# YangGuang001/siddhi

Hardware: AMD Instinct MI355X
Metric: input events/sec (node) for partitioned pattern query; achieved HBM GB/s % (higher is better)
Workload: dtype f32+i64

## Files before the change

### siddhi_amd/abi.py

```python
import ctypes as C

SH_DESC_VERSION = 5
SH_MAX_ORDER = 4
SH_MAX_GROUP = 4

SH_OK = 0
SH_E_INVALID_ARG = -1
SH_E_OOM = -2
SH_E_HIP = -3
SH_E_UNSUPPORTED = -4
SH_E_STATE_OVERFLOW = -5
SH_E_MORE = -6
SH_E_NO_DEVICE = -7

STATUS_NAMES = {0: "OK", -1: "INVALID_ARG", -2: "OOM", -3: "HIP", -4: "UNSUPPORTED",
                -5: "STATE_OVERFLOW", -6: "MORE", -7: "NO_DEVICE"}


class sh_expr(C.Structure):
    _fields_ = [("op", C.c_int32), ("type", C.c_int32), ("lhs", C.c_int32), ("rhs", C.c_int32),
                ("third", C.c_int32), ("ltype", C.c_int32), ("rtype", C.c_int32),
                ("slot", C.c_int32), ("chain", C.c_int32), ("attr", C.c_int32),
                ("is_null", C.c_int32), ("pad", C.c_int32), ("cval", C.c_int64)]

# ... 59 lines not shown


class sh_due_cand(C.Structure):
    _fields_ = [("t", C.c_int64), ("order", C.c_uint64), ("key", C.c_int32), ("pad", C.c_int32)]


HISTORY_FN = C.CFUNCTYPE(C.c_int, C.c_void_p, C.POINTER(C.c_uint64), C.c_int64,
                         C.POINTER(C.POINTER(C.c_uint64)), C.POINTER(C.c_int64))
SELECT_FN = C.CFUNCTYPE(C.c_int, C.c_void_p, C.c_int32, C.POINTER(sh_due_cand), C.c_int64,
                        C.POINTER(C.c_int64), C.POINTER(C.c_int64))
MIN_TIME_FN = C.CFUNCTYPE(C.c_int, C.c_void_p, C.c_int64, C.POINTER(C.c_int64))


class sh_coordinator(C.Structure):
    _fields_ = [("user", C.c_void_p), ("history", HISTORY_FN), ("select", SELECT_FN), ("min_time", MIN_TIME_FN)]


class sh_kernel_times(C.Structure):
    _fields_ = [("segment_ms", C.c_float), ("advance_ms", C.c_float), ("emit_ms", C.c_float),
                ("total_ms", C.c_float), ("advance_launches", C.c_int64)]


EXPORTED = ["sh_start", "sh_compile", "sh_push_batch", "sh_advance_time", "sh_drain", "sh_pending",
            "sh_destroy", "sh_last_error", "sh_run_device", "sh_run_device_v2", "sh_last_kernel_times",
            "sh_version", "sh_device_count", "sh_set_partition_keys", "sh_snapshot", "sh_restore",
            "sh_set_coordinator", "sh_push_batch_part", "sh_drain_ordered", "sh_list_get",
            "sh_packed_row_layout"]


def bind_product(lib):
    lib.sh_compile.argtypes = [C.POINTER(sh_app_desc), C.POINTER(C.c_void_p)]
    lib.sh_compile.restype = C.c_int
    lib.sh_start.argtypes = [C.c_void_p]
    lib.sh_start.restype = C.c_int
    lib.sh_push_batch.argtypes = [C.c_void_p, C.POINTER(sh_batch)]
    lib.sh_push_batch.restype = C.c_int
    lib.sh_advance_time.argtypes = [C.c_void_p, C.c_int64]
    lib.sh_advance_time.restype = C.c_int
    lib.sh_drain.argtypes = [C.c_void_p, C.POINTER(sh_match_buf)]
    lib.sh_drain.restype = C.c_int
    lib.sh_pending.argtypes = [C.c_void_p]
    lib.sh_pending.restype = C.c_int64
    lib.sh_destroy.argtypes = [C.c_void_p]
    lib.sh_destroy.restype = None
    lib.sh_last_error.argtypes = [C.c_void_p]
    lib.sh_last_error.restype = C.c_char_p
    lib.sh_set_partition_keys.argtypes = [C.c_void_p, C.c_int32, C.c_int32, C.c_void_p, C.c_void_p]
    lib.sh_set_partition_keys.restype = C.c_int
    lib.sh_run_device.argtypes = [C.c_void_p, C.POINTER(sh_device_run)]
    lib.sh_run_device.restype = C.c_int
    lib.sh_run_device_v2.argtypes = [C.c_void_p, C.POINTER(sh_device_run)]
    lib.sh_run_device_v2.restype = C.c_int
    lib.sh_last_kernel_times.argtypes = [C.c_void_p, C.POINTER(sh_kernel_times)]
    lib.sh_last_kernel_times.restype = C.c_int
    lib.sh_packed_row_layout.argtypes = [C.c_void_p, C.POINTER(C.c_int32), C.c_int32, C.POINTER(C.c_int32),
                                         C.POINTER(C.c_int32)]
    lib.sh_packed_row_layout.restype = C.c_int
    lib.sh_snapshot.argtypes = [C.c_void_p, C.c_void_p, C.c_int64, C.POINTER(C.c_int64)]
    lib.sh_snapshot.restype = C.c_int
    lib.sh_restore.argtypes = [C.c_void_p, C.c_void_p, C.c_int64]
    lib.sh_restore.restype = C.c_int
    lib.sh_set_coordinator.argtypes = [C.c_void_p, C.POINTER(sh_coordinator)]
    lib.sh_set_coordinator.restype = C.c_int
    lib.sh_push_batch_part.argtypes = [C.c_void_p, C.POINTER(sh_batch), C.c_void_p, C.c_int64, C.c_int64]
    lib.sh_push_batch_part.restype = C.c_int
    lib.sh_drain_ordered.argtypes = [C.c_void_p, C.POINTER(sh_match_buf), C.c_void_p]
    lib.sh_drain_ordered.restype = C.c_int
    lib.sh_list_get.argtypes = [C.c_void_p, C.c_int64, C.c_int64, C.c_void_p, C.c_void_p]
    lib.sh_list_get.restype = C.c_int64
    lib.sh_version.argtypes = []
    lib.sh_version.restype = C.c_char_p
    lib.sh_device_count.argtypes = []
    lib.sh_device_count.restype = C.c_int
    lib.shx_jit_status.argtypes = [C.c_void_p]
    lib.shx_jit_status.restype = C.c_int
    lib.shx_jit_compile.argtypes = [C.c_void_p]
    lib.shx_jit_compile.restype = C.c_int
    lib.shx_jit_source.argtypes = [C.c_void_p, C.c_char_p, C.c_int64]
    lib.shx_jit_source.restype = C.c_int64
    lib.shx_bucket_compile.argtypes = [C.c_void_p, C.c_char_p, C.c_int64]
    lib.shx_bucket_compile.restype = C.c_int
    lib.shx_bucket_status.argtypes = [C.c_void_p]
    lib.shx_bucket_status.restype = C.c_int
    lib.shx_bucket_emit_status.argtypes = [C.c_void_p]
    lib.shx_bucket_emit_status.restype = C.c_int
    lib.shx_emit_compile.argtypes = [C.c_void_p, C.c_int, C.c_char_p, C.c_int64]
    lib.shx_emit_compile.restype = C.c_int
    lib.shx_emit_compile_key.argtypes = [C.POINTER(C.c_int32), C.c_char_p, C.c_int64, C.c_char_p, C.c_int64]
    lib.shx_emit_compile_key.restype = C.c_int
    lib.shx_seq3_status.argtypes = [C.c_void_p]
    lib.shx_seq3_status.restype = C.c_int
    lib.shx_agg_status.argtypes = [C.c_void_p]
    lib.shx_agg_status.restype = C.c_int
    lib.shx_having_status.argtypes = [C.c_void_p]
    lib.shx_having_status.restype = C.c_int
    lib.shx_having_rows.argtypes = [C.c_void_p, C.POINTER(C.c_int64), C.POINTER(C.c_int64)]
    lib.shx_having_rows.restype = C.c_int
    lib.shx_having_ms.argtypes = [C.c_void_p]
    lib.shx_having_ms.restype = C.c_double
    lib.shx_rate_status.argtypes = [C.c_void_p]
    lib.shx_rate_status.restype = C.c_int
    lib.shx_rate_rows.argtypes = [C.c_void_p, C.POINTER(C.c_int64), C.POINTER(C.c_int64)]
    lib.shx_rate_rows.restype = C.c_int
    lib.shx_rate_ms.argtypes = [C.c_void_p]
    lib.shx_rate_ms.restype = C.c_double
    lib.shx_fingerprint.argtypes = [C.c_void_p]
    lib.shx_fingerprint.restype = C.c_uint64
    lib.shx_rules_status.argtypes = [C.c_void_p]
    lib.shx_rules_status.restype = C.c_int
    lib.shx_rules_carry.argtypes = [C.c_void_p, C.POINTER(C.c_int64), C.POINTER(C.c_int64)]
    lib.shx_rules_carry.restype = C.c_int
    lib.shx_rules_agg_carry.argtypes = [C.c_void_p, C.POINTER(C.c_int64)]
    lib.shx_rules_agg_carry.restype = C.c_int
    lib.shx_rules_agg_capacity.argtypes = [C.c_void_p]
    lib.shx_rules_agg_capacity.restype = C.c_int64
    lib.shx_host_profile.argtypes = [C.c_void_p, C.c_void_p, C.c_void_p, C.c_int]
    lib.shx_host_profile.restype = C.c_int
    lib.shx_seq3_shape.argtypes = [C.c_void_p]
    lib.shx_seq3_shape.restype = C.c_int
    return lib


def bind_oracle(lib):
    lib.ref_create.argtypes = [C.POINTER(sh_app_desc), C.c_char_p, C.c_int]
    lib.ref_create.restype = C.c_void_p
    lib.ref_start.argtypes = [C.c_void_p]
    lib.ref_start.restype = None
    lib.ref_send.argtypes = [C.c_void_p, C.POINTER(sh_batch), C.c_uint64]
    lib.ref_send.restype = C.c_int
    lib.ref_set_partition_keys.argtypes = [C.c_void_p, C.c_int32, C.c_int32, C.c_void_p, C.c_void_p]
    lib.ref_set_partition_keys.restype = C.c_int
    lib.ref_advance_time.argtypes = [C.c_void_p, C.c_int64]
    lib.ref_advance_time.restype = C.c_int
    lib.ref_out_count.argtypes = [C.c_void_p]
    lib.ref_out_count.restype = C.c_int64
    lib.ref_out_read.argtypes = [C.c_void_p, C.c_int64, C.c_int64, C.c_void_p, C.c_void_p,
                                 C.c_void_p, C.c_void_p, C.c_void_p, C.c_int32, C.c_void_p]
    lib.ref_out_read.restype = C.c_int
    lib.ref_out_clear.argtypes = [C.c_void_p]
    lib.ref_out_clear.restype = None
    lib.ref_list_get.argtypes = [C.c_void_p, C.c_int64, C.c_int64, C.c_void_p, C.c_void_p]
    lib.ref_list_get.restype = C.c_int64
    lib.ref_destroy.argtypes = [C.c_void_p]
    lib.ref_destroy.restype = None
    return lib


def object_columns(compiled):
    return [[k for k, t in enumerate(q.out_types) if t == 6] for q in compiled.queries]


def resolve_lists(out, obj_cols, get):
    import numpy as np
    lists = {}
    if any(obj_cols):
        q = out["query"]
        for r in range(len(q)):
            cols = obj_cols[int(q[r])] if 0 <= int(q[r]) < len(obj_cols) else []
            for c in cols:
                if not out["nulls"][r, c]:
                    v, nl = get(int(out["values"][r, c]))
                    lists[(r, c)] = (np.asarray(v, np.int64), np.asarray(nl, np.uint8))
    out["lists"] = lists
    return out


# ... 26 lines not shown
```

### siddhi_amd/build.py

```python
import os
import subprocess
import sys

HERE = os.path.dirname(os.path.abspath(__file__))
CSRC = os.path.join(HERE, "csrc")
OUT = os.path.join(HERE, "libsiddhi_hip.so")
SOURCES = ["sh_host.cpp", "sh_host_nfa.cpp", "sh_host_fast.cpp", "sh_host_snap.cpp", "sh_jit.cpp", "sh_nfa_lower.cpp", "sh_kernels.hip", "sh_window.hip", "sh_nfa.hip", "sh_rules.hip", "sh_bucket.hip", "sh_shard.hip", "sh_agg.hip", "sh_having.hip", "sh_rate.hip"]
JIT_HEADERS = [os.path.join(HERE, "..", "include", "sh_query.h"), os.path.join(CSRC, "sh_program.h"),
               os.path.join(CSRC, "sh_device.h"), os.path.join(CSRC, "sh_vm.h"),
               os.path.join(CSRC, "sh_wave.h")]
JIT_EMIT_HEADERS = [os.path.join(CSRC, "sh_rows.h"), os.path.join(CSRC, "sh_bk_emit.h")]
JIT_INC = os.path.join(CSRC, "sh_jit_src.inc")
JIT_PRELUDE = """typedef __hip_internal::int8_t int8_t;
typedef __hip_internal::uint8_t uint8_t;
typedef __hip_internal::int16_t int16_t;
typedef __hip_internal::uint16_t uint16_t;
typedef __hip_internal::int32_t int32_t;
typedef __hip_internal::uint32_t uint32_t;
typedef __hip_internal::int64_t int64_t;
typedef __hip_internal::uint64_t uint64_t;
typedef decltype(sizeof(0)) size_t;
#define INT32_MIN (-2147483647 - 1)
#define INT64_MIN (-9223372036854775807LL - 1)
"""
FLAGS = ["-O3", "-std=c++17", "-fPIC", "-shared", "--offload-arch=gfx950", "-ffp-contract=off",
         "-fno-gpu-flush-denormals-to-zero", "-fhip-fp32-correctly-rounded-divide-sqrt",
         "-Wall", "-Wno-unused-function", "-Wno-unused-result", "-Wno-unused-value", "-L/opt/rocm/lib", "-lhiprtc", "-Wl,-rpath,/opt/rocm/lib"]


def _jit_text(headers, prelude=""):
    parts = [prelude]
    for h in headers:
        with open(h) as f:
            for line in f:
                t = line.strip()
                if t.startswith("#include") or t == "#pragma once":
                    continue
                parts.append(line)
    text = "".join(parts)
    assert ')SHJ"' not in text
    return text


def write_jit_inc():
    inc = "// generated by siddhi_amd/build.py from the device headers -- do not edit\n" \
          "static const char SHJ_HEADERS[] = R\"SHJ(" + _jit_text(JIT_HEADERS, JIT_PRELUDE) + ")SHJ\";\n" \
          "static const char SHJ_EMIT_SRC[] = R\"SHJ(" + _jit_text(JIT_EMIT_HEADERS) + ")SHJ\";\n"
    if os.path.exists(JIT_INC) and open(JIT_INC).read() == inc:
        return
    with open(JIT_INC, "w") as f:
        f.write(inc)


def needs_build():
    if not os.path.exists(OUT):
        return True
    t = os.path.getmtime(OUT)
    deps = [os.path.join(CSRC, f) for f in os.listdir(CSRC)] + \
        [os.path.join(HERE, "..", "include", f) for f in os.listdir(os.path.join(HERE, "..", "include"))]
    return any(os.path.getmtime(d) > t for d in deps)


OBJ_DIR = os.path.join(HERE, "build")
COMPILE_FLAGS = [f for f in FLAGS if f not in ("-shared",) and not f.startswith(("-L", "-l", "-Wl"))]
LINK_FLAGS = ["-shared", "-fPIC", "--offload-arch=gfx950", "-L/opt/rocm/lib", "-lhiprtc", "-Wl,-rpath,/opt/rocm/lib"]


def _headers_mtime():
    hs = [os.path.join(CSRC, f) for f in os.listdir(CSRC) if f.endswith((".h", ".inc"))] + \
        [os.path.join(HERE, "..", "include", f) for f in os.listdir(os.path.join(HERE, "..", "include"))]
    return max(os.path.getmtime(h) for h in hs)


def build(force=False, verbose=False):
    write_jit_inc()
    if not force and not needs_build():
        return OUT
    from concurrent.futures import ThreadPoolExecutor
    hipcc = os.environ.get("HIPCC", "/opt/rocm/bin/hipcc")
    os.makedirs(OBJ_DIR, exist_ok=True)
    hmt = _headers_mtime()
    objs, jobs = [], []
    for src in SOURCES:
        sp = os.path.join(CSRC, src)
        op = os.path.join(OBJ_DIR, src + ".o")
        objs.append(op)
        if force or not os.path.exists(op) or os.path.getmtime(op) < max(os.path.getmtime(sp), hmt):
            jobs.append([hipcc] + COMPILE_FLAGS + ["-c", sp, "-o", op])

    def run(cmd):
        if verbose:
            print(" ".join(cmd), file=sys.stderr)
# ... 14 lines not shown
```

### siddhi_amd/csrc/sh_bk_emit.h

```cpp
#pragma once
#include <hip/hip_runtime.h>
#include <stdint.h>

#include "../../include/sh_query.h"
#include "sh_device.h"
#include "sh_rows.h"
#include "sh_wave.h"

#define BK_TPB 512
#define BK_ITEMS (SHB_TILE / BK_TPB)

static_assert(BK_ITEMS == 16, "tile / threads");


__device__ __forceinline__ int bk_tile(int nt) {
    const int per = (nt + 7) >> 3;
    const int t = (int)(blockIdx.x & 7u) * per + (int)(blockIdx.x >> 3);
    return t < nt ? t : -1;
}
__device__ __forceinline__ int bk_tile(int t0, int t1) {
    const int t = bk_tile(t1 - t0);
    return t < 0 ? -1 : t0 + t;
}

// ... 23 lines not shown
        bk_vals<NO>(O, i, mp, row, v);
        bk_store<MODE, NO>(OC, row, v, seq, out_seq, out_vals);
        return;
    }
#ifndef BKS_NO
    const int no = O.n_out;
    if (MODE == SHB_OUT_PACKED) {
        uint32_t* r = (uint32_t*)OC.rows + row * OC.rw;
        r[0] = (uint32_t)seq;
        r[1] = (uint32_t)(seq >> 32);
        for (int k = 2; k < OC.rw; k++) r[k] = 0u;
    } else if (out_seq) {
        out_seq[row] = seq;
    }
    for (int o = 0; o < no; o++) {
        const int64_t v = bk_raw(o_src[o], o_kind[o] == 1 ? i : mp, o_type[o]);
        if (MODE == SHB_OUT_PACKED) {
            uint32_t* r = (uint32_t*)OC.rows + row * OC.rw + OC.woff[o];
            r[0] = OC.colw[o] == 1 ? (uint32_t)(uint8_t)v : (uint32_t)v;
            if (OC.colw[o] == 8) r[1] = (uint32_t)((uint64_t)v >> 32);
        } else if (MODE == SHB_OUT_COLS) {
            bk_put(OC.cols[o], OC.colw[o], row, v);
        } else if (out_vals) {
            out_vals[row * no + o] = v;
        }
    }
#endif
}

#ifdef BKS_NO
extern "C" __global__ void __launch_bounds__(BK_TPB, BKS_OCC) BKS_NAME(shb_plan P, bks_ptrs Q, uint64_t seq_base,
                                                               uint64_t* __restrict__ out_seq,
                                                               int64_t* __restrict__ out_vals, int64_t out_cap) {
    constexpr int MODE = BKS_MODE, NO = BKS_NO, BK_RU = BKS_RU, BK_OCC = BKS_OCC;
    const bks_ptrs &O = Q, &OC = Q;
#else
template <int MODE, int NO, int BK_RU, int BK_OCC = 4>
__global__ void __launch_bounds__(BK_TPB, BK_OCC) k_bk_emit(shb_plan P, shb_out O, shb_cols OC, uint64_t seq_base,
                                                    uint64_t* __restrict__ out_seq, int64_t* __restrict__ out_vals,
                                                    int64_t out_cap) {
#endif
    constexpr bool LM = BK_OCC >= 6;
    constexpr int EROWS = LM ? 512 : BK_EROWS;
    constexpr int EMPW = LM ? 2 * BK_EHALF : BK_EHALF;
    constexpr int BK_MAPW = (BK_TPB / 64) * (EROWS / 2 + EMPW + BK_EHALF / 2);
    __shared__ uint32_t pool[(SHB_TILE + 1) > BK_MAPW ? (SHB_TILE + 1) : BK_MAPW];
    uint32_t* const pfx = pool;
    uint16_t(*const rmap)[EROWS] = (uint16_t(*)[EROWS])pool;
    uint32_t(*const emp)[EMPW] = (uint32_t(*)[EMPW])(pool + (BK_TPB / 64) * (EROWS / 2));
    uint16_t(*const ero)[BK_EHALF] =
        (uint16_t(*)[BK_EHALF])(pool + (BK_TPB / 64) * (EROWS / 2 + EMPW));
    __shared__ uint32_t ms0[SHB_NB];
    __shared__ uint16_t to[SHB_NB + 1];
    __shared__ uint32_t wtot[BK_TPB / 64], ws[BK_TPB / 64];
    __shared__ int32_t o_kind[SHB_MAX_OUT], o_type[SHB_MAX_OUT];
    __shared__ const void* o_src[SHB_MAX_OUT];
    __shared__ uint32_t s_tb;
    constexpr int NV = NO > 0 ? NO : 1;
    const int T = bk_tile(P.et0, P.et1);
    if (T < 0) return;
    const int64_t b0 = (int64_t)T << SHB_TILE_SHIFT;
    const int tile_n = (int)((P.n - b0) < SHB_TILE ? (P.n - b0) : SHB_TILE);
    const int lane = threadIdx.x & 63, w = threadIdx.x >> 6;
    if (threadIdx.x <= SHB_NB) to[threadIdx.x] = P.toff[(int64_t)T * SHB_TOFF + threadIdx.x];
    if (threadIdx.x < SHB_NB) ms0[threadIdx.x] = P.mstart[(int64_t)T * SHB_NB + threadIdx.x];
    if (threadIdx.x == 0) s_tb = P.ttot[T];
#ifndef BKS_NO
    if (NO == 0 && threadIdx.x < SHB_MAX_OUT) {
#pragma unroll
        for (int o = 0; o < SHB_MAX_OUT; o++)
            if (o == (int)threadIdx.x) {
                o_kind[o] = O.kind[o];
                o_type[o] = O.type[o];
                o_src[o] = O.src[o];
            }
    }
#endif
    uint32_t sl[BK_ITEMS];
    {
        const int l0 = w * (64 * BK_ITEMS) + lane;
#pragma unroll
        for (int j = 0; j < BK_ITEMS; j++) {
            const int l = l0 + j * 64;
            sl[j] = l < tile_n ? (uint32_t)P.sp[b0 + l] : BK_NOSLOT;
        }
    }
    {
        const int s0 = threadIdx.x * 16;
        const uint4 q = *(const uint4*)(P.cnt + b0 + s0);
        __syncthreads();
        const int nv = to[SHB_NB];
        uint32_t c[16];
        const uint32_t wd[4] = {q.x, q.y, q.z, q.w};
        uint32_t sum = 0;
#pragma unroll
        for (int k = 0; k < 16; k++) {
            c[k] = (s0 + k < nv) ? (wd[k >> 2] >> (8 * (k & 3))) & 0xFFu : 0u;
            sum += c[k];
        }
        uint32_t tot;
        uint32_t off = shw_block_excl<BK_TPB>(sum, ws, &tot);
        int d = 0;
        {
            int lo = 0, hi = SHB_NB - 1;
            while (lo < hi) {
                const int mid = (lo + hi + 1) >> 1;
                if ((int)to[mid] <= s0) lo = mid;
                else hi = mid - 1;
            }
            d = lo;
        }
#pragma unroll
        for (int k = 0; k < 16; k++) {
            while (d < SHB_NB - 1 && (int)to[d + 1] <= s0 + k) d++;
            pfx[s0 + k] = off | ((uint32_t)d << BK_PFX_BITS);
            off += c[k];
        }
        if (threadIdx.x == 0) pfx[SHB_TILE] = tot;
        __syncthreads();
    }
    uint32_t cp[BK_ITEMS / 4];
    uint32_t mp[BK_ITEMS];
    uint32_t mine = 0;
#pragma unroll
    for (int j = 0; j < BK_ITEMS; j++) {
        uint32_t c = 0;
        mp[j] = 0u;
        if (sl[j] != BK_NOSLOT) {
            const uint32_t s = sl[j];
            const uint32_t pw = pfx[s];
            const uint32_t d = pw >> BK_PFX_BITS;
            const uint32_t ps = pw & BK_PFX_MASK;
            c = (pfx[s + 1] & BK_PFX_MASK) - ps;
            mp[j] = ms0[d] + ps - (pfx[to[d]] & BK_PFX_MASK);
        }
        if ((j & 3) == 0) cp[j >> 2] = 0u;
        cp[j >> 2] |= c << (8 * (j & 3));
        mine += c;
    }
    {
        const uint32_t wsum = shw_last(shw_incl_scan(mine));
        if (lane == 0) wtot[w] = wsum;
    }
    __syncthreads();
    if (LM) {
#pragma unroll
        for (int j = 0; j < BK_ITEMS; j++) emp[w][j * 64 + lane] = mp[j];
    }
    uint64_t rb = s_tb;
    for (int q = 0; q < w; q++) rb += wtot[q];
#pragma unroll
    for (int hf = 0; hf < BK_ITEMS / 8; hf++) {
        uint32_t carry = 0;
        uint32_t ro8[8];
#pragma unroll
        for (int jj = 0; jj < 8; jj++) {
            const int j = hf * 8 + jj;
            const uint32_t c = (cp[j >> 2] >> (8 * (j & 3))) & 0xFFu;
            const uint32_t incl = shw_incl_scan(c);
            const uint32_t ro = carry + incl - c;
            if (!LM) ro8[jj] = ro;
            const int e = jj * 64 + lane;
            if (!LM) emp[w][e] = mp[j];
            ero[w][e] = (uint16_t)ro;
            for (uint32_t k = 0; k < c; k++)
                if (ro + k < EROWS) rmap[w][ro + k] = (uint16_t)e;
            carry += shw_last(incl);
// ... 74 lines not shown
```

### siddhi_amd/csrc/sh_bucket.hip

```cpp
#include <hip/hip_runtime.h>
#include <stdlib.h>
#include <string.h>

#include "../../include/sh_query.h"
#include "sh_device.h"
#include "sh_nfa.h"
#include "sh_bk_emit.h"
#include "sh_rows.h"
#include "sh_wave.h"

static inline unsigned bk_grid(int nt) { return 8u * (unsigned)((nt + 7) >> 3); }


template <int MINW, int TPB>
__global__ void __launch_bounds__(TPB, MINW) k_bk_scatter(const int32_t* __restrict__ keys,
                                                          const int64_t* __restrict__ ts, int32_t nkeys, shb_plan P) {
    constexpr int SC_ITEMS = SHB_TILE / TPB;
    __shared__ uint32_t wcnt[TPB / 64][256];
    __shared__ uint32_t tstart[256];
    __shared__ uint32_t ws[TPB / 64];
    __shared__ uint32_t stage[SHB_TILE];
    __shared__ int64_t s_tmx[TPB / 64];
    const int T = bk_tile(P.nt);
    if (T < 0) return;
    const int64_t b0 = (int64_t)T << SHB_TILE_SHIFT;
    const int lane = threadIdx.x & 63, w = threadIdx.x >> 6;
    for (int c = threadIdx.x; c < (TPB / 64) * 256; c += TPB) (&wcnt[0][0])[c] = 0u;
    __syncthreads();
    int32_t key[SC_ITEMS];
    uint32_t rw[SC_ITEMS], wp[SC_ITEMS];
    const uint64_t lt = lane ? (~0ull >> (64 - lane)) : 0ull;
    {
        int64_t tv[SC_ITEMS];
        const int64_t e0 = b0 + (int64_t)w * (64 * SC_ITEMS) + lane;
        if (b0 + SHB_TILE <= P.n) {
            const int32_t* __restrict__ pk = keys + e0;
            const int64_t* __restrict__ pt = ts + e0;
#pragma unroll
            for (int j = 0; j < SC_ITEMS; j++) {
                key[j] = pk[j * 64];
                tv[j] = pt[j * 64];
            }
        } else {
#pragma unroll
            for (int j = 0; j < SC_ITEMS; j++) {
                const int64_t i = e0 + j * 64;
                const bool in = i < P.n;
                key[j] = in ? keys[i] : -1;
                tv[j] = in ? ts[i] : P.tbase;
            }
        }
        const int64_t lim = (int64_t)1 << (32 - P.kb);
        bool bad = false, badk = false;
        int64_t tmx = INT64_MIN;
#pragma unroll
        for (int j = 0; j < SC_ITEMS; j++) {
            const int64_t dt = tv[j] - P.tbase;
            if (key[j] >= nkeys) badk = true;
            if (key[j] >= 0 && !P.no_ts && (dt < 0 || dt >= lim)) bad = true;
            if (key[j] >= 0 && tv[j] > tmx) tmx = tv[j];
            wp[j] = P.no_ts ? ((uint32_t)key[j] >> 8) : (((uint32_t)dt << P.kb) | ((uint32_t)key[j] >> 8));
            rw[j] = key[j] >= 0 ? ((uint32_t)key[j] & (SHB_NB - 1)) << 16 : ~0u;
        }
        if (bad) atomicOr(P.flag, SHB_F_TS);
        if (badk) atomicOr(P.flag, SHB_F_KEY);
#pragma unroll
        for (int o = 32; o >= 1; o >>= 1) {
            const int64_t y = __shfl_xor(tmx, o);
            tmx = y > tmx ? y : tmx;
        }
        if (lane == 0) s_tmx[w] = tmx;
        if (threadIdx.x == 0) P.tfirst[T] = tv[0];
    }
    {
        uint32_t old[SC_ITEMS];
#pragma unroll
        for (int j = 0; j < SC_ITEMS; j++) {
            const bool valid = rw[j] != ~0u;
            const uint32_t d = (rw[j] >> 16) & (SHB_NB - 1);
            uint64_t peers = __ballot(valid);
#pragma unroll
            for (int bb = 0; bb < 8; bb++) {
                const bool bit = (d >> bb) & 1u;
                const uint64_t m = __ballot(valid && bit);
                peers &= bit ? m : ~m;
            }
            const uint32_t r = (uint32_t)__popcll(peers & lt);
            old[j] = 0u;
            if (valid && r == 0) old[j] = atomicAdd(&wcnt[w][d], (uint32_t)__popcll(peers));
            rw[j] = valid ? (r | ((uint32_t)(__ffsll((unsigned long long)peers) - 1) << 8) | (d << 16)) : ~0u;
        }
#pragma unroll
        for (int j = 0; j < SC_ITEMS; j++) {
            const uint32_t ld = rw[j] == ~0u ? (uint32_t)lane : (rw[j] >> 8) & 63u;
            const uint32_t base = (uint32_t)__shfl((int)old[j], (int)ld);
            if (rw[j] != ~0u) rw[j] = ((base + (rw[j] & 0xFFu)) & 0xFFFFu) | (rw[j] & 0xFF0000u);
        }
    }
    __syncthreads();
    uint32_t nvalid;
    {
        uint32_t tot = 0;
        if (threadIdx.x < 256) {
#pragma unroll
            for (int q = 0; q < TPB / 64; q++) {
                const uint32_t c = wcnt[q][threadIdx.x];
                wcnt[q][threadIdx.x] = tot;
                tot += c;
            }
        }
        const uint32_t ex = shw_block_excl<TPB>(threadIdx.x < 256 ? tot : 0u, ws, &nvalid);
        if (threadIdx.x < 256) {
            tstart[threadIdx.x] = ex;
            P.toff[(int64_t)T * SHB_TOFF + threadIdx.x] = (uint16_t)ex;
        }
        if (threadIdx.x == 256) P.toff[(int64_t)T * SHB_TOFF + 256] = (uint16_t)nvalid;
        if (threadIdx.x == 0) {
            int64_t m = s_tmx[0];
#pragma unroll
            for (int q = 1; q < TPB / 64; q++) m = s_tmx[q] > m ? s_tmx[q] : m;
            P.tpre[T] = m;
        }
    }
    __syncthreads();
#pragma unroll
    for (int j = 0; j < SC_ITEMS; j++) {
        const bool valid = rw[j] != ~0u;
        const uint32_t d = (rw[j] >> 16) & (SHB_NB - 1);
        rw[j] = valid ? tstart[d] + wcnt[w][d] + (rw[j] & 0xFFFFu) : ~0u;
        const int64_t i = b0 + (int64_t)w * (64 * SC_ITEMS) + j * 64 + lane;
        if (i < P.n) P.sp[i] = (uint16_t)rw[j];
        if (valid) stage[rw[j]] = wp[j];
    }
    __syncthreads();
    const int64_t ob = (int64_t)T << SHB_TILE_SHIFT;
#define BK_WRITE_OUT(TY, DST, EXPR)                                                  \
    {                                                                                \
        _Pragma("unroll 4") for (int m = 0; m < SC_ITEMS; m++) {                     \
            const uint32_t l = (uint32_t)(m * TPB + threadIdx.x);                 \
            if (l < nvalid) ((TY*)(DST))[EXPR(ob + l)] = (TY)stage[l];               \
        }                                                                            \
        __syncthreads();                                                             \
    }
#define BK_ID(x) (x)
#define BK_LO(x) (2 * (x))
#define BK_HI(x) (2 * (x) + 1)
    BK_WRITE_OUT(uint32_t, P.w0, BK_ID);
    for (int c = 0; c < P.n_staged; c++) {
        const int wd = P.st_width[c];
        const int halves = wd == 8 ? 2 : 1;
        for (int hh = 0; hh < halves; hh++) {
#pragma unroll
            for (int j = 0; j < SC_ITEMS; j++) {
                if (rw[j] == ~0u) continue;
                const int64_t i = b0 + (int64_t)w * (64 * SC_ITEMS) + j * 64 + lane;
                uint32_t v;
                if (wd == 8) v = ((const uint32_t*)P.st_src[c])[2 * i + hh];
                else if (wd == 4) v = ((const uint32_t*)P.st_src[c])[i];
                else v = ((const uint8_t*)P.st_src[c])[i];
                stage[rw[j]] = v;
            }
            __syncthreads();
            if (wd == 8) {
                if (hh == 0) BK_WRITE_OUT(uint32_t, P.st_dst[c], BK_LO)
                else BK_WRITE_OUT(uint32_t, P.st_dst[c], BK_HI)
            } else if (wd == 4) {
                BK_WRITE_OUT(uint32_t, P.st_dst[c], BK_ID)
            } else {
                BK_WRITE_OUT(uint8_t, P.st_dst[c], BK_ID)
            }
        }
    }
#undef BK_WRITE_OUT
#undef BK_ID
#undef BK_LO
#undef BK_HI
}


__device__ __forceinline__ void bk_halo(const int64_t* __restrict__ tfirst, int32_t* __restrict__ hstart, int32_t nt,
                                        int64_t within, int t) {
    if (t >= nt) return;
    const int64_t ta = tfirst[t];
    const int64_t tlim = ta < INT64_MIN + within ? INT64_MIN : ta - within;
    int h = t > 0 ? 1 : 0;
    while (h < t && h < SHB_HMAX && tfirst[t - h] >= tlim) h++;
    hstart[t] = t - h;
}

__device__ __forceinline__ void bk_tpre(int64_t* __restrict__ tpre, int32_t nt, int64_t* s) {
    const int per = (nt + 1023) / 1024;
    const int t0 = threadIdx.x * per;
    int64_t m = INT64_MIN;
    for (int t = t0; t < t0 + per && t < nt; t++) m = tpre[t] > m ? tpre[t] : m;
    s[threadIdx.x] = m;
    __syncthreads();
    for (int o = 1; o < 1024; o <<= 1) {
        const int64_t y = threadIdx.x >= (unsigned)o ? s[threadIdx.x - o] : INT64_MIN;
        __syncthreads();
        if (y > s[threadIdx.x]) s[threadIdx.x] = y;
        __syncthreads();
    }
    int64_t run = threadIdx.x ? s[threadIdx.x - 1] : INT64_MIN;
    for (int t = t0; t < t0 + per && t < nt; t++) {
        const int64_t v = tpre[t];
        tpre[t] = run;
        run = v > run ? v : run;
    }
}

#define S3B_TPB 1024
#define S3B_CH 4096
#define S3B_NR (S3B_CH / S3B_TPB)
#define S3B_NK 4096
#define S3B_W (S3B_TPB / 64)

__device__ __forceinline__ NfVal s3b_val(uint32_t b, int t) {
    NfVal v;
    v.t = (uint8_t)t;
    v.null = 0;
    v.b = t == SH_T_INT ? (int64_t)(int32_t)b : (int64_t)b;
    return v;
}

__device__ __forceinline__ void s3b_sort_pass(const uint32_t* __restrict__ c_key, const uint16_t* in,
                                              uint16_t* out, int L, int sh, uint32_t (*wc)[64], uint32_t* ws) {
    const int lane = threadIdx.x & 63, w = threadIdx.x >> 6;
    const uint64_t lt = lane ? (~0ull >> (64 - lane)) : 0ull;
    for (int c = threadIdx.x; c < S3B_W * 64; c += S3B_TPB) (&wc[0][0])[c] = 0u;
    __syncthreads();
    uint32_t rk[S3B_NR], dg[S3B_NR], ix[S3B_NR];
#pragma unroll
    for (int r = 0; r < S3B_NR; r++) {
        const int pos = (w * S3B_NR + r) * 64 + lane;
        const bool valid = pos < L;
        ix[r] = valid ? (in ? (uint32_t)in[pos] : (uint32_t)pos) : 0u;
        const uint32_t d = valid ? (c_key[ix[r]] >> sh) & 63u : 0u;
        uint64_t peers = __ballot(valid);
#pragma unroll
        for (int bb = 0; bb < 6; bb++) {
            const bool bit = (d >> bb) & 1u;
            const uint64_t m = __ballot(valid && bit);
            peers &= bit ? m : ~m;
        }
        const uint32_t r_ = (uint32_t)__popcll(peers & lt);
        const uint32_t base = valid ? wc[w][d] : 0u;
        if (valid && r_ == 0) wc[w][d] = base + (uint32_t)__popcll(peers);
        rk[r] = valid ? base + r_ : ~0u;
        dg[r] = d;
    }
    __syncthreads();
    {
        const int d = threadIdx.x >> 4, q = threadIdx.x & 15;
        uint32_t tot;
        const uint32_t ex = shw_block_excl<S3B_TPB>(wc[q][d], ws, &tot);
        __syncthreads();
        wc[q][d] = ex;
    }
    __syncthreads();
#pragma unroll
    for (int r = 0; r < S3B_NR; r++)
        if (rk[r] != ~0u) out[wc[w][dg[r]] + rk[r]] = (uint16_t)ix[r];
    __syncthreads();
}

__device__ __forceinline__ void s3b_sort_pass8(const uint32_t* __restrict__ c_key, uint16_t* out, int L,
                                               uint32_t (*wc8)[256], uint32_t* ws) {
    const int lane = threadIdx.x & 63, w = threadIdx.x >> 6;
    const uint64_t lt = lane ? (~0ull >> (64 - lane)) : 0ull;
    for (int c = threadIdx.x; c < S3B_W * 256; c += S3B_TPB) (&wc8[0][0])[c] = 0u;
    __syncthreads();
    uint32_t rk[S3B_NR], dg[S3B_NR];
#pragma unroll
    for (int r = 0; r < S3B_NR; r++) {
        const int pos = (w * S3B_NR + r) * 64 + lane;
        const bool valid = pos < L;
        const uint32_t d = valid ? c_key[pos] & 255u : 0u;
        uint64_t peers = __ballot(valid);
#pragma unroll
        for (int bb = 0; bb < 8; bb++) {
            const bool bit = (d >> bb) & 1u;
            const uint64_t m = __ballot(valid && bit);
            peers &= bit ? m : ~m;
        }
        const uint32_t r_ = (uint32_t)__popcll(peers & lt);
        const uint32_t base = valid ? wc8[w][d] : 0u;
        if (valid && r_ == 0) wc8[w][d] = base + (uint32_t)__popcll(peers);
        rk[r] = valid ? base + r_ : ~0u;
        dg[r] = d;
    }
// ... 602 lines not shown
                type[o] = SH_T_INT;
                mode[o] = o < A.n ? agp_mode(A, o, &type[o]) : 2;
            }
            bool bad = false;
            for (int ri = wv; ri < nruns; ri += AGC_TPB / 64) {
                const int q0 = run_q[ri], q1 = run_q[ri + 1];
                const int R0 = rs[q0], R1 = rs[q1];
                const uint32_t key = c_key[srt[q0]] & 0xFFFFu;
                int64_t acc[SHB_MAX_AGG];
#pragma unroll
                for (int o = 0; o < SHB_MAX_AGG; o++) acc[o] = st_acc[o][key];
                const int64_t n0 = st_cnt[key];
                for (int r0 = R0; r0 < R1; r0 += 64) {
                    const int r = r0 + lane;
                    const bool ok = r < R1;
                    uint32_t mp = 0u, gi = 0u, wp = 0u;
                    int64_t x1 = 0, x2 = 0, x3 = 0;
                    if (ok) {
                        const uint32_t q = rq[r];
                        const uint32_t cr = srt[q];
                        const uint32_t m = (uint32_t)(r - rs[q]);
                        mp = c_mp[cr] + m;
                        wp = mp;
                        gi = c_gi[cr];
                        if (e1src) x1 = (int64_t)e1src[mp];
                        if (e2src) x2 = agc_load(e2src, gi, A.e2_type[0]);
                        if (e2srn) x3 = (int64_t)e2srn[gi];
                    }
                    const int64_t n = n0 + (r + 1 - R0);
#pragma unroll
                    for (int o = 0; o < SHB_MAX_AGG; o++) {
                        if (o >= A.n) break;
                        int64_t* out = (int64_t*)A.out[o];
                        if (mode[o] == 2) {
                            if (ok) out[wp] = n;
                            continue;
                        }
                        const int sd = A.side[o];
                        int64_t u = 0;
                        if (ok) bad |= !agp_units(mode[o], type[o], sd == 0 ? x1 : (sd == 1 ? x2 : x3), &u);
                        u = (int64_t)shw_incl_scan64((uint64_t)u);
                        const int64_t v = (int64_t)((uint64_t)acc[o] + (uint64_t)u);
                        if (ok) {
                            if (mode[o] == 0) {
                                out[wp] = v;
                            } else {
                                double d = (double)v;
                                bad |= fabs(d) >= AGP_LIM;
                                if (type[o] == SH_T_FLOAT || type[o] == SH_T_DOUBLE) d *= 5.9604644775390625e-08;
                                if (A.kind[o] == SH_AGG_AVG) d = d / (double)n;
                                out[wp] = __double_as_longlong(d);
                            }
                        }
                        acc[o] = (int64_t)(((uint64_t)(uint32_t)__builtin_amdgcn_readlane((int)((uint64_t)v >> 32), 63) << 32) |
                                           (uint32_t)__builtin_amdgcn_readlane((int)v, 63));
                    }
                }
                if (lane == 0) {
#pragma unroll
                    for (int o = 0; o < SHB_MAX_AGG; o++) st_acc[o][key] = acc[o];
                    st_cnt[key] = n0 + (R1 - R0);
                }
            }
            if (bad) s_bad = 1;
        }
        __syncthreads();
        if (s_bad) {
            if (threadIdx.x == 0) atomicOr(P.flag, SHB_F_AGG);
            return;
        }
        AGP_PROF(3)
        a += ne;
    }
#undef AGP_PROF
}

static int bk_ok() { return hipGetLastError() == hipSuccess ? 0 : -3; }

#define TT_T 64
__global__ void __launch_bounds__(1024) k_bk_prep_a(const uint16_t* __restrict__ toff, int nt,
                                                    uint16_t* __restrict__ tofft, int stride,
                                                    uint32_t* __restrict__ tpfx, uint32_t* __restrict__ tpfb, int nbt,
                                                    const int64_t* __restrict__ tfirst, int32_t* __restrict__ hstart,
                                                    int64_t within) {
    __shared__ uint16_t s[TT_T][SHB_NB + 2];
    if ((int)blockIdx.x >= nbt) {
        bk_halo(tfirst, hstart, nt, within, ((int)blockIdx.x - nbt) * 1024 + (int)threadIdx.x);
        return;
    }
    const int T0 = (int)blockIdx.x * TT_T;
    for (int i = threadIdx.x; i < TT_T * (SHB_NB + 1); i += 1024) {
        const int t = i / (SHB_NB + 1), b = i - t * (SHB_NB + 1);
        s[t][b] = T0 + t < nt ? toff[(int64_t)(T0 + t) * SHB_TOFF + b] : (uint16_t)0;
    }
    __syncthreads();
    static_assert(TT_T == 64, "a tile per lane");
    const int t = (int)(threadIdx.x & 63u);
    for (int b = (int)(threadIdx.x >> 6); b < SHB_NB + 1; b += 1024 / 64) {
        const uint32_t lo = s[t][b];
        if (T0 + t < nt) tofft[(int64_t)b * stride + T0 + t] = (uint16_t)lo;
        if (tpfx && b < SHB_NB) {
            const uint32_t len = (uint32_t)s[t][b + 1] - lo;
            const uint32_t incl = shw_incl_scan(len);
            if (T0 + t < stride) tpfx[(int64_t)b * stride + T0 + t] = incl - len;
            if (t == 63) tpfb[(int64_t)b * (nbt + 1) + blockIdx.x] = incl;
        }
    }
}

__global__ void __launch_bounds__(1024) k_bk_prep_b(uint32_t* __restrict__ tpfb, int nbt, int64_t* __restrict__ tpre,
                                                    int32_t nt, int ntp) {
    __shared__ int64_t s[1024];
    if ((int)blockIdx.x < ntp) {
        bk_tpre(tpre, nt, s);
        return;
    }
    const int b = ((int)blockIdx.x - ntp) * (1024 / 64) + (int)(threadIdx.x >> 6), lane = (int)(threadIdx.x & 63u);
    if (b >= SHB_NB) return;
    uint32_t* row = tpfb + (int64_t)b * (nbt + 1);
    uint32_t carry = 0;
    for (int base = 0; base <= nbt; base += 64) {
        const int i = base + lane;
        const uint32_t v = i < nbt ? row[i] : 0u;
        const uint32_t incl = shw_incl_scan(v);
        if (i <= nbt) row[i] = carry + incl - v;
        carry += shw_last(incl);
    }
}

extern "C" int shb_partition(const int32_t* keys, const int64_t* ts, int32_t nkeys, shb_plan* P, void* stream) {
    hipStream_t st = (hipStream_t)stream;
    hipLaunchKernelGGL((k_bk_scatter<2, 1024>), dim3(bk_grid(P->nt)), dim3(1024), 0, st, keys, ts, nkeys, *P);
    if (bk_ok()) return -3;
    if (P->tstride < P->nt) return -1;
    const int nbt = (P->nt + TT_T - 1) / TT_T, ntp = P->no_ts ? 0 : 1;
    const bool pfx = P->tpfx && P->tpfb;
    if (pfx && P->tstride != nbt * TT_T) return -1;
    hipLaunchKernelGGL(k_bk_prep_a, dim3(nbt + (P->no_ts ? 0 : (P->nt + 1023) / 1024)), dim3(1024), 0, st,
                       (const uint16_t*)P->toff, P->nt, P->tofft, P->tstride, pfx ? P->tpfx : nullptr,
                       pfx ? P->tpfb : nullptr, nbt, P->tfirst, P->hstart, P->within);
    if (ntp || pfx)
        hipLaunchKernelGGL(k_bk_prep_b, dim3(ntp + (pfx ? SHB_NB / (1024 / 64) : 0)), dim3(1024), 0, st, P->tpfb, nbt,
                           P->tpre, P->nt, ntp);
    return bk_ok();
}

extern "C" int shb_finish(shb_plan* P, uint32_t* scan_tmp, void* stream) {
    return shd_exclusive_scan(P->ttot, P->ttot, (int64_t)P->nt + 1, scan_tmp, stream);
}

#define BK_SEG_TPB 1024
__global__ void __launch_bounds__(BK_SEG_TPB) k_bk_scan_seg(uint32_t* __restrict__ ttot, int32_t t0, int32_t t1,
                                                            int32_t nt, uint32_t* __restrict__ carry, int32_t last) {
    __shared__ uint32_t ws[BK_SEG_TPB / 64];
    const int per = (t1 - t0 + BK_SEG_TPB - 1) / BK_SEG_TPB;
    const int a = t0 + (int)threadIdx.x * per, e = a + per < t1 ? a + per : t1;
    uint32_t s = 0;
    for (int t = a; t < e; t++) s += ttot[t];
    uint32_t tot;
    uint32_t off = shw_block_excl<BK_SEG_TPB>(s, ws, &tot) + *carry;
    for (int t = a; t < e; t++) {
        const uint32_t v = ttot[t];
        ttot[t] = off;
        off += v;
    }
    __syncthreads();
    if (threadIdx.x == 0) {
        const uint32_t c = *carry + tot;
        *carry = c;
        if (last) ttot[nt] = c;
    }
}

extern "C" int shb_finish_seg(shb_plan* P, int32_t t0, int32_t t1, uint32_t* carry, int last, void* stream) {
    if (t0 < 0 || t0 >= t1 || t1 > P->nt) return -1;
    hipLaunchKernelGGL(k_bk_scan_seg, dim3(1), dim3(BK_SEG_TPB), 0, (hipStream_t)stream, P->ttot, t0, t1, P->nt, carry,
                       last);
    return bk_ok();
}

extern "C" int shb_s3_carry(const shb_plan* P, const shb_s3* S, void* stream) {
    if (P->kb > 12 || P->n_staged < 1 || P->st_width[0] != 4) return -1;
    hipLaunchKernelGGL(k_s3b, dim3(SHB_NB), dim3(S3B_TPB), 0, (hipStream_t)stream, *P, *S);
    return bk_ok();
}

extern "C" int shb_agg_carry(const shb_plan* P, const shb_aggc* A, void* stream) {
    static_assert(AGC_TPB == S3B_TPB && AGC_CH == S3B_CH, "the sort pass shape");
    if (P->kb > 8 || A->n < 1 || A->n > SHB_MAX_AGG) return -1;
    if (A->parallel)
        hipLaunchKernelGGL(k_bk_aggp, dim3(SHB_NB), dim3(AGC_TPB), 0, (hipStream_t)stream, *P, *A);
    else
        hipLaunchKernelGGL(k_bk_aggc, dim3(SHB_NB), dim3(AGC_TPB), 0, (hipStream_t)stream, *P, *A);
    return bk_ok();
}

template <int MODE, int NO>
constexpr int bk_ru_lm() {
    return NO == 0 ? 4
         : MODE == SHB_OUT_COLS ? (NO <= 2 ? 4 : 0)
                                : (NO <= 3 ? 4 : NO == 4 ? 3 : NO == 5 ? 2 : 0);
}

template <int MODE, int NO>
static void bk_emit_launch(const shb_plan* P, const shb_out* O, const shb_cols& OC, uint64_t seq_base,
                           uint64_t* out_seq, int64_t* out_vals, int64_t out_cap, void* stream) {
    constexpr int RL = bk_ru_lm<MODE, NO>();
    if constexpr (RL > 0) {
        hipLaunchKernelGGL((k_bk_emit<MODE, NO, RL, 6>), dim3(bk_grid(P->et1 - P->et0)), dim3(BK_TPB), 0, (hipStream_t)stream,
                           *P, *O, OC, seq_base, out_seq, out_vals, out_cap);
        return;
    }
    constexpr int RU = (NO >= 1 && NO <= 4) ? (MODE == SHB_OUT_COLS && NO == 4 ? 4 : 6)
                                            : (MODE == SHB_OUT_RAW ? (NO <= 6 ? 4 : 3)
                                                                   : (MODE == SHB_OUT_PACKED ? (NO <= 6 ? 4 : (NO == 7 ? 2 : 1))
                                                                                             : (NO <= 5 ? 2 : 1)));
    hipLaunchKernelGGL((k_bk_emit<MODE, NO, RU>), dim3(bk_grid(P->et1 - P->et0)), dim3(BK_TPB), 0, (hipStream_t)stream, *P,
                       *O, OC, seq_base, out_seq, out_vals, out_cap);
}

template <int MODE>
static void bk_emit_width(const shb_plan* P, const shb_out* O, const shb_cols& OC, uint64_t seq_base,
                          uint64_t* out_seq, int64_t* out_vals, int64_t out_cap, void* stream) {
    switch (O->n_out) {
        case 1: bk_emit_launch<MODE, 1>(P, O, OC, seq_base, out_seq, out_vals, out_cap, stream); break;
        case 2: bk_emit_launch<MODE, 2>(P, O, OC, seq_base, out_seq, out_vals, out_cap, stream); break;
// ... 117 lines not shown
```

### siddhi_amd/csrc/sh_device.h

```cpp
#pragma once
#include <stddef.h>
#include <stdint.h>

#include "sh_program.h"

#define SHD_NULL_ROW 0xFFFFFFFFu

struct shd_cols {
    const void* col[SHP_MAX_STREAMS][32];
    const uint8_t* nul[SHP_MAX_STREAMS][32];
};

struct shd_batch {
    const int64_t* ts;
    const uint8_t* stream;
    const uint32_t* row;
    const int32_t* keys;
    uint32_t row_base;
    int32_t pad;
    uint64_t seq_base;
    int64_t n;
};

struct shd_emit {
    uint64_t* tmp;
    unsigned long long* tmp_ctr;
    int64_t tmp_cap;
    uint32_t* match_cnt;
    int32_t* err;
};

struct shd_segment_ws {
    uint32_t* keys_a;
    uint32_t* keys_b;
    uint32_t* idx_a;
    uint32_t* idx_b;
    uint32_t* hist;
    uint32_t* scan_tmp;
    uint32_t* seg_off;
    int64_t cap;
};

struct shd_payload {
    int32_t n;
    int32_t pad;
    const void* src[8];
    void* dst[8];
    uint8_t width[8];
};

struct shd_tiles {
    const uint32_t* dstart;
    const uint32_t* dend;
    uint32_t K1;
    uint32_t ntile;
    int32_t shift;
    int32_t pad;
};

struct shd_window_ws {
    int32_t* match_pos;
    uint32_t* cnt_s;
    uint32_t* cnt;
    uint32_t* off;
    int32_t* flag;
};

#define SHB_NB 256
#define SHB_TILE_SHIFT 13
#define SHB_TILE (1 << SHB_TILE_SHIFT)
#define SHB_CH 4096
#define SHB_SPAN 5120
#define SHB_TOFF 264
#define SHB_HMAX 64
#define SHB_CT_MAX 160
#define SHB_MAX_STAGED 4
#define SHB_MAX_MS 4
#define SHB_MAX_OUT 16
#define SHB_F_TS 1
#define SHB_F_KEY 2
#define SHB_F_MONO 4
#define SHB_F_COUNT 8
#define SHB_F_HALO 16
#define SHB_F_SPAN 32

struct shb_plan {
    int64_t n;
    int64_t tbase;
    int32_t nt;
    int32_t kb;
    int32_t ct;
    int32_t n_chunks;
    int32_t n_staged;
    int32_t no_ts;
    const void* st_src[SHB_MAX_STAGED];
    void* st_dst[SHB_MAX_STAGED];
    int32_t st_width[SHB_MAX_STAGED];
    int32_t n_ms;
    void* ms[SHB_MAX_MS];
    int32_t ms_width[SHB_MAX_MS];
    const int64_t* ts;
    const int32_t* keys;
    uint32_t* w0;
    uint16_t* sp;
    uint16_t* toff;
    uint16_t* tofft;
    int32_t tstride;
    int32_t c0;
    int32_t et0, et1;
    int32_t pad_t;
    uint32_t* tpfx;
    uint32_t* tpfb;
    uint8_t* cnt;
    uint32_t* mstart;
    uint32_t* ttot;
    uint32_t* ms_ctr;
    int64_t* tpre;
    int64_t* tfirst;
    int32_t* hstart;
    int64_t within;
    int32_t* flag;
    unsigned long long* prof;
};

struct shb_out {
    int32_t n_out;
    int32_t pad[3];
    int32_t kind[SHB_MAX_OUT];
    int32_t type[SHB_MAX_OUT];
    const void* src[SHB_MAX_OUT];
};

struct shb_s3 {
    int32_t type;
    int32_t op2, dom2, op3, dom3;
    int32_t n_ms;
    int32_t ms_slot[2];
    int32_t warm;
};

#define SHB_MAX_AGG 4
#define SHB_F_AGG 64
struct shb_aggc {
    int32_t n;
    int32_t e1_col, e1_type;
    int32_t e2_col[2], e2_type[2];
    int32_t kind[SHB_MAX_AGG];
    int32_t side[SHB_MAX_AGG];
    void* out[SHB_MAX_AGG];
    int32_t parallel;
};

#define SHB_OUT_RAW 0
#define SHB_OUT_COLS 1
#define SHB_OUT_PACKED 2
struct shb_cols {
    void* cols[SHB_MAX_OUT];
    int32_t colw[SHB_MAX_OUT];
    int32_t use;
    int32_t rw;
    int32_t woff[SHB_MAX_OUT];
    void* rows;
};

#ifdef __cplusplus
extern "C" {
#endif
size_t shd_scan_tmp_words(int64_t n);
int shd_segment(const shd_batch* b, int32_t nkeys, shd_segment_ws* ws, void* stream,
                const uint32_t** perm_out, const uint32_t** skeys_out);
int shd_segment_payload(const shd_batch* b, int32_t nkeys, shd_segment_ws* ws, void* stream,
                        const uint32_t** perm_out, const uint32_t** skeys_out, const shd_payload* carry,
                        void* const* mid, int tile_shift, int want_segments);
int shd_advance(const shp_program* dprog, const shp_layout* lay, uint8_t* kstate, int32_t nkeys,
                const shd_batch* b, const uint32_t* perm, const uint32_t* skeys,
                const uint32_t* seg_off, const shd_cols* dcols, const shd_emit* em, void* stream, int fast_ok);
int shd_emit_place(const shd_emit* em, int32_t n_out, int64_t n_events, uint32_t* offsets,
                   uint32_t* scan_tmp, int64_t n_records, const shd_batch* b, uint64_t* out_seq,
                   int64_t* out_ts, int64_t* out_vals, uint8_t* out_nulls, void* stream);
int shd_window(const shp_program* dprog, const shp_program* hprog, const shd_batch* b, int32_t nkeys,
               const uint32_t* perm, const uint32_t* skeys, const int64_t* sts, const void* const* scols,
               shd_window_ws* ws, shd_cols* d_sorted_desc, uint32_t* scan_tmp, uint64_t* out_seq,
               int64_t* out_ts, int64_t* out_vals, uint8_t* out_nulls, int64_t out_cap, int64_t* n_matches,
               void* stream, void* ev_mid, const void* jit, const shd_tiles* tiles);
int shd_tile_dir(const uint32_t* skeys, int64_t n, int shift, uint32_t K1, uint32_t ntile, uint32_t* ds,
                 uint32_t* de, void* stream);
int shd_relayout(const uint8_t* src, const shp_layout* A, uint8_t* dst, const shp_layout* B, int32_t nkeys,
                 int32_t n_states, int32_t n_out, void* stream);
int shd_sort_pairs(const uint32_t* keys, const uint32_t* vals, int64_t n, int bits, uint32_t* const* kbuf,
                   uint32_t* const* vbuf, uint32_t* hist, uint32_t* scan_tmp, void* stream,
                   const uint32_t** keys_out, const uint32_t** vals_out);
int shd_exclusive_scan(const uint32_t* in, uint32_t* out, int64_t n, uint32_t* tmp, void* stream);
int shb_partition(const int32_t* keys, const int64_t* ts, int32_t nkeys, shb_plan* P, void* stream);
int shb_finish(shb_plan* P, uint32_t* scan_tmp, void* stream);
int shb_finish_seg(shb_plan* P, int32_t t0, int32_t t1, uint32_t* carry, int last, void* stream);
int shb_s3_carry(const shb_plan* P, const shb_s3* S, void* stream);
int shb_agg_carry(const shb_plan* P, const shb_aggc* A, void* stream);
int shb_emit(const shb_plan* P, const shb_out* O, const shb_cols* OC, uint64_t seq_base, uint64_t* out_seq,
             int64_t* out_vals, int64_t out_cap, void* stream);
int shb_emit_spec(void* fn, const shb_plan* P, const shb_out* O, const shb_cols* OC, uint64_t seq_base,
                  uint64_t* out_seq, int64_t* out_vals, int64_t out_cap, void* stream);
int shd_narrow_rows(const int64_t* vals, int32_t n_out, int64_t m, void* const* cols, const int32_t* w, void* stream);
int shd_pack_rows(const uint64_t* seq, const int64_t* vals, int32_t n_out, int64_t m, const int32_t* w,
                  const int32_t* woff, int32_t rw, void* rows, void* stream);
#ifdef __cplusplus
}
#endif
```

### siddhi_amd/csrc/sh_host.cpp

```cpp
#include "sh_host_int.h"

#define SH_VERSION_STR "siddhi_hip 0.2 (gfx950; sh_device_run layout 2)"

namespace {

struct Lowering {
    const sh_query_desc* q;
    shp_program P;
    std::string err;
    std::vector<int> chain;

    int add_const(int64_t v, int type, int isnull) {
        for (int i = 0; i < P.n_const; i++)
            if (P.consts[i] == v && P.const_type[i] == type && P.const_null[i] == isnull) return i;
        if (P.n_const >= 64) {
            err = "too many constants";
            return -1;
        }
        P.consts[P.n_const] = v;
        P.const_type[P.n_const] = (uint8_t)type;
        P.const_null[P.n_const] = (uint8_t)isnull;
        return P.n_const++;
    }
    bool emit(uint8_t op, uint8_t a, uint8_t b, uint8_t c, int32_t x) {
// ... 1606 lines not shown
static void packed_layout(const int32_t* w, int n_out, int32_t* woff, int32_t* rw) {
    int pos = 2;
    for (int o = 0; o < n_out; o++) {
        const int wd = w[o] == 8 ? 2 : 1;
        if (wd == 2 && (pos & 1)) pos++;
        woff[o] = pos;
        pos += wd;
    }
    *rw = (pos + 3) & ~3;
}

int sh_packed_row_layout(sh_handle* h, int32_t* offsets, int32_t cap, int32_t* n_out, int32_t* row_bytes) {
    if (!h || !n_out || !row_bytes) return SH_E_INVALID_ARG;
    int32_t w[SHB_MAX_OUT], woff[SHB_MAX_OUT], rw = 0;
    const int rc = out_widths(h, w, "packed rows");
    if (rc) return rc;
    packed_layout(w, h->n_out, woff, &rw);
    for (int o = 0; o < h->n_out && offsets && o < cap; o++) offsets[o] = woff[o] * 4;
    *n_out = h->n_out;
    *row_bytes = rw * 4;
    return SH_OK;
}

static int run_device_cols(sh_handle* h, sh_device_run* run) {
    if (run->out_layout != SH_OUT_RAW && run->out_layout != SH_OUT_PACKED)
        return fail(h, SH_E_INVALID_ARG, "sh_device_run.out_layout");
    const bool packed = run->out_layout == SH_OUT_PACKED;
    if (packed && run->d_out_cols) return fail(h, SH_E_INVALID_ARG, "packed rows and typed columns together");
    if (packed && !run->d_out_values) return fail(h, SH_E_INVALID_ARG, "packed rows: d_out_values is NULL");
    if (!run->d_out_cols && !packed) return run_device_impl(h, run);
    int32_t w[SHB_MAX_OUT];
    {
        const int wrc = out_widths(h, w, packed ? "packed rows" : "typed columns");
        if (wrc) return wrc;
    }
    h->out_mode = packed ? SHB_OUT_PACKED : SHB_OUT_COLS;
    if (packed) {
        for (int o = 0; o < h->n_out; o++) h->pk_w[o] = w[o];
        packed_layout(w, h->n_out, h->pk_woff, &h->pk_rw);
    }
    int64_t* user_vals = run->d_out_values;
    uint64_t* user_seq = run->d_out_seq;
    h->cols_rows = false;
    int rc = run_device_impl(h, run);
    if (h->cols_rows) {
        if (rc == SH_OK && run->out_count > 0) {
            const int64_t m = std::min(run->out_count, run->out_capacity);
            const int crc = packed ? shd_pack_rows(h->w_packseq.as<uint64_t>(), h->w_colrows.as<int64_t>(), h->n_out, m,
                                                   w, h->pk_woff, h->pk_rw, user_vals, h->stream)
                                   : shd_narrow_rows(h->w_colrows.as<int64_t>(), h->n_out, m, run->d_out_cols, w,
                                                     h->stream);
            if (crc || hipStreamSynchronize(h->stream) != hipSuccess)
                rc = fail(h, SH_E_HIP, packed ? "packed-row conversion failed" : "typed-column narrowing failed");
        }
        h->cols_rows = false;
    }
    h->out_mode = SHB_OUT_RAW;
    run->d_out_values = user_vals;
    run->d_out_seq = user_seq;
    return rc;
}

int shx_jit_status(sh_handle* h) { return h ? h->jit_state : 0; }

int shx_jit_compile(sh_handle* h) {
    if (!h) return SH_E_INVALID_ARG;
    shj_window w;
    std::string err;
    if (!h->prog.window_ok) return fail(h, SH_E_UNSUPPORTED, "not a window-shaped program");
    if (shj_window_compile(&h->prog, &w, &err)) return fail(h, SH_E_HIP, err);
    return SH_OK;
}

int shx_bucket_status(sh_handle* h) {
    if (!h) return 0;
    if (h->bk_state == -2) return 0;
    if (h->bk_state < 0) {
        h->err = h->bk_err;
        return -1;
    }
    return h->bk_last;
}

int shx_bucket_emit_status(sh_handle* h) {
    if (!h) return 0;
    if (h->bk_emit_last < 0) h->err = h->bk_emit_err;
    return h->bk_emit_last;
}

int shx_seq3_status(sh_handle* h) { return h ? (h->s3b_last ? 2 : h->seq3_last) : 0; }
int shx_agg_status(sh_handle* h) { return h ? h->agg_last : 0; }

int shx_having_status(sh_handle* h) { return h ? h->hv.last : 0; }
int shx_having_rows(sh_handle* h, int64_t* rows_in, int64_t* rows_kept) {
    return h ? h->hv.rows(rows_in, rows_kept) : 0;
}
double shx_having_ms(sh_handle* h) { return h ? h->hv.ms() : 0.0; }

int shx_rate_status(sh_handle* h) { return h ? h->rl.last : 0; }
int shx_rate_rows(sh_handle* h, int64_t* rows_in, int64_t* rows_kept) {
    return h ? h->rl.rows(rows_in, rows_kept) : 0;
}
double shx_rate_ms(sh_handle* h) { return h ? h->rl.ms() : 0.0; }

uint64_t shx_fingerprint(sh_handle* h) { return h ? h->fp : 0; }

int shx_rules_status(sh_handle* h) { return h ? h->rs_last : 0; }

int shx_rules_carry(sh_handle* h, int64_t* partials, int64_t* rows) {
    if (!h) return 0;
    if (partials) *partials = h->rc_pairs;
    if (rows) *rows = h->rc_rows;
    return (int)std::min<int64_t>(h->rc_steps, 0x7FFFFFFF);
}

int shx_rules_agg_carry(sh_handle* h, int64_t* entries) {
    if (!h) return 0;
    if (entries) *entries = h->ag_tab.entries;
    return (int)std::min<int64_t>(h->ag_tab.entries, 0x7FFFFFFF);
}
int64_t shx_rules_agg_capacity(sh_handle* h) { return h ? h->ag_tab.cap : 0; }

int shx_host_profile(sh_handle* h, double* ms, int64_t* n, int cap) {
    if (!h) return 0;
    const int k = cap < SH_HP_N ? cap : SH_HP_N;
    for (int i = 0; i < k; i++) {
        if (ms) ms[i] = h->hp_ms[i];
        if (n) n[i] = h->hp_n[i];
    }
    return SH_HP_N;
}
int shx_seq3_shape(sh_handle* h) { return h && h->T && h->T->n_queries == 1 && h->T->q[0].s3 ? 1 : 0; }

int shx_bucket_compile(sh_handle* h, char* buf, int64_t len) {
    if (!h) return SH_E_INVALID_ARG;
    const shp_program& P = h->prog;
    if (!P.window_ok || !P.out_fast) return fail(h, SH_E_UNSUPPORTED, "not a window-shaped projection");
    int ms[SHB_MAX_MS], n_ms = 0;
    for (int o = 0; o < P.n_out; o++) {
        const int a = P.out_attr[o], t = P.attr_type[0][a];
        const bool fold = a == h->part_attr0 && (t == SH_T_STRING || t == SH_T_INT || t == SH_T_LONG || t == SH_T_BOOL);
        if (P.out_slot[o] == 1 || fold) continue;
        int m = 0;
        while (m < n_ms && ms[m] != a) m++;
        if (m == n_ms && n_ms < SHB_MAX_MS) ms[n_ms++] = a;
    }
    std::string src, err;
    if (shj_bucket_source(&P, ms, n_ms, &src)) return fail(h, SH_E_UNSUPPORTED, "no consumer-side form");
    if (buf && len > 0) {
        const int64_t k = std::min<int64_t>(len - 1, (int64_t)src.size());
        memcpy(buf, src.data(), k);
        buf[k] = 0;
    }
    if (shj_bucket_compile(&P, ms, n_ms, &err)) return fail(h, SH_E_HIP, err);
    return SH_OK;
}

static void copy_text(const std::string& t, char* buf, int64_t len) {
    if (!buf || len <= 0) return;
    const int64_t k = std::min<int64_t>(len - 1, (int64_t)t.size());
    memcpy(buf, t.data(), k);
    buf[k] = 0;
}

int shx_emit_compile(sh_handle* h, int layout, char* buf, int64_t len) {
    if (!h) return SH_E_INVALID_ARG;
// ... 56 lines not shown
```

### siddhi_amd/csrc/sh_host_fast.cpp

```cpp
#include "sh_host_int.h"

int bits_for(uint64_t v) {
    int b = 0;
    while (b < 64 && (v >> b)) b++;
    return b;
}

shd_segment_ws seg_ws(sh_handle* h, int64_t n) {
    shd_segment_ws ws;
    ws.keys_a = h->w_keys_a.as<uint32_t>();
    ws.keys_b = h->w_keys_b.as<uint32_t>();
    ws.idx_a = h->w_idx_a.as<uint32_t>();
    ws.idx_b = h->w_idx_b.as<uint32_t>();
    ws.hist = h->w_hist.as<uint32_t>();
    ws.scan_tmp = h->w_scan.as<uint32_t>();
    ws.seg_off = h->w_seg.as<uint32_t>();
    ws.cap = n;
    return ws;
}

int carry_setup(sh_handle* h, const sh_device_run* run, shd_payload* carry, void** mid, int* alias,
                       bool used_only, bool with_ts) {
    const int64_t n = run->n;
    const int na = (int)h->stream_types[0].size();
// ... 898 lines not shown
        hipMemsetAsync(ctl.p, 0, 16, st);
        arc = shc_put(&T, post.put_keys, post.put_state, ml, ctl.as<unsigned long long>(), ctl.as<int32_t>() + 2, st);
        hipMemcpyAsync(rl_ctl, ctl.p, 16, hipMemcpyDeviceToHost, st);
    }
    if (shr_klast_update(sts, skeys, perm, n, (uint32_t)nc, h->rc_klast.as<int64_t>(), st) || arc ||
        (hipEventRecord(h->ev[3], st), hipStreamSynchronize(st)) != hipSuccess || (ag_ctl[1] & 1) ||
        (rl_ctl[1] & 1)) {
        out_queue_rows(h, base);
        return rules_step_fail(h, SH_E_HIP, "device error in the rule step");
    }
    phase_times(h);
    h->rc_cur = 1 - h->rc_cur;
    h->rc_rows = nrows;
    h->rc_pairs = npairs;
    h->rc_steps++;
    h->rs_last = 0;
    if (ag_pk) h->ag_tab.entries += (int64_t)ag_ctl[0];
    if (h->r_aggp) h->agg_last = 6;
    h->hv.last = h->hv_on ? 1 : 0;
    h->hv.rows_in = m;
    h->hv.rows_kept = ml;
    if (post.put_keys) h->rl_tab.entries += (int64_t)rl_ctl[0];
    h->rl.last = h->rl_on ? 1 : 0;
    h->rl.rows_in = ml;
    h->rl.rows_kept = mk;
    rules_unstage(h);
    return SH_OK;
}

shd_batch device_batch(const sh_handle* h, const sh_device_run* run) {
    return shd_batch{run->d_ts, nullptr, nullptr, h->partitioned ? run->d_keys : nullptr, 0, 0, 0, run->n};
}

void phase_times(sh_handle* h) {
    hipEventElapsedTime(&h->times.segment_ms, h->ev[0], h->ev[1]);
    hipEventElapsedTime(&h->times.advance_ms, h->ev[1], h->ev[2]);
    hipEventElapsedTime(&h->times.emit_ms, h->ev[2], h->ev[3]);
    hipEventElapsedTime(&h->times.total_ms, h->ev[0], h->ev[3]);
}


static int bk_workspace(sh_handle* h, const sh_device_run* run, int kb, bool matcher, const char* oom, shb_plan* B) {
    const int64_t n = run->n;
    B->n = n;
    B->nt = (int32_t)((n + SHB_TILE - 1) / SHB_TILE);
    B->et1 = B->nt;
    B->kb = kb;
    B->no_ts = matcher ? 0 : 1;
    B->tstride = (B->nt + 63) & ~63;
    const int64_t nt = B->nt, slots = nt * SHB_TILE;
    if (ensure_ws(h, matcher ? std::max(n, nt + 1) : nt + 1) || h->bk_w0.ensure_fresh(slots * 4) ||
        h->bk_sp.ensure_fresh(n * 2) || h->bk_toff.ensure_fresh(nt * SHB_TOFF * 2) || h->bk_cnt.ensure_fresh(slots) ||
        h->bk_mstart.ensure_fresh(nt * SHB_NB * 4) || h->bk_tpre.ensure_fresh(nt * 8) ||
        h->bk_tfirst.ensure_fresh(nt * 8) || h->bk_hstart.ensure_fresh(nt * 4) ||
        h->bk_ttot.ensure_fresh((nt + 1) * 4) || h->bk_flag.ensure_fresh(64) || h->bk_rd.ensure(64) ||
        h->bk_tofft.ensure_fresh((int64_t)(SHB_NB + 1) * B->tstride * 2) ||
        (matcher && (h->bk_tpfx.ensure_fresh((int64_t)SHB_NB * B->tstride * 4) ||
                     h->bk_tpfb.ensure_fresh((int64_t)SHB_NB * (B->tstride / 64 + 1) * 4))))
        return fail(h, SH_E_OOM, oom);
    B->ts = run->d_ts;
    B->keys = run->d_keys;
    B->w0 = h->bk_w0.as<uint32_t>();
    B->sp = h->bk_sp.as<uint16_t>();
    B->toff = h->bk_toff.as<uint16_t>();
    B->tofft = h->bk_tofft.as<uint16_t>();
    B->tpfx = matcher ? h->bk_tpfx.as<uint32_t>() : nullptr;
    B->tpfb = matcher ? h->bk_tpfb.as<uint32_t>() : nullptr;
    B->cnt = h->bk_cnt.as<uint8_t>();
    B->mstart = h->bk_mstart.as<uint32_t>();
    B->tpre = h->bk_tpre.as<int64_t>();
    B->tfirst = h->bk_tfirst.as<int64_t>();
    B->hstart = h->bk_hstart.as<int32_t>();
    B->ttot = h->bk_ttot.as<uint32_t>();
    B->flag = h->bk_flag.as<int32_t>();
    B->ms_ctr = h->bk_flag.as<uint32_t>() + 4;
    if (shj_bucket_profiled()) {
        if (h->bk_prof.ensure_fresh(128)) return fail(h, SH_E_OOM, "profile");
        hipMemsetAsync(h->bk_prof.p, 0, 128, h->stream);
        B->prof = h->bk_prof.as<unsigned long long>();
    }
    return SH_OK;
}

static int bk_begin(sh_handle* h, const sh_device_run* run, int32_t nkeys, shb_plan* B, const char* what) {
    hipStream_t st = h->stream;
    hipEventRecord(h->ev[0], st);
    hipMemsetAsync(B->flag, 0, 32, st);
    hipMemsetAsync(B->ttot, 0, ((int64_t)B->nt + 1) * 4, st);
    if (shb_partition(run->d_keys, run->d_ts, nkeys, B, st)) return fail(h, SH_E_HIP, what);
    hipEventRecord(h->ev[1], st);
    return SH_OK;
}

static int bk_end(sh_handle* h, const shb_plan* B, const char* what, int32_t* flag, int64_t* total) {
    hipStream_t st = h->stream;
    hipEventRecord(h->ev[3], st);
    hipMemcpyAsync(h->bk_rd.as<void>(0), B->flag, 4, hipMemcpyDeviceToHost, st);
    hipMemcpyAsync(h->bk_rd.as<void>(8), B->ttot + B->nt, 4, hipMemcpyDeviceToHost, st);
    if (hipStreamSynchronize(st) != hipSuccess) return fail(h, SH_E_HIP, what);
    *flag = *h->bk_rd.as<int32_t>(0);
    *total = *h->bk_rd.as<uint32_t>(8);
    return SH_OK;
}

static int bk_close(sh_handle* h, sh_device_run* run, int32_t flag, int64_t total, int* last, const char* what) {
    hipStream_t st = h->stream;
    if (flag & SHB_F_KEY) return fail(h, SH_E_INVALID_ARG, "partition key id >= n_keys");
    if (flag) return 1;
    run->out_count = total;
    if (total > run->out_capacity) return fail(h, SH_E_MORE, "output capacity too small");
    if (run->d_out_query && total > 0) hipMemsetAsync(run->d_out_query, 0, total * 4, st);
    phase_times(h);
    h->times.advance_launches = 1;
    *last = 1;
    return hipStreamSynchronize(st) == hipSuccess ? SH_OK : fail(h, SH_E_HIP, what);
}

static void* bk_emit_fn(sh_handle* h, const shb_out& O, const shb_cols& OC) {
    h->bk_emit_last = 0;
    if (const char* e = getenv("SH_BK_EMIT_SPEC"))
        if (atoi(e) == 0) return nullptr;
    shj_emit_key K;
    if (shj_emit_key_of(&O, &OC, &K)) return nullptr;
    const sh_handle::BkEmit* hit = nullptr;
    for (const auto& c : h->bk_emit)
        if (!memcmp(&c.key, &K, sizeof(K))) hit = &c;
    if (!hit) {
        void* fn = nullptr;
        if (shj_emit_load(&K, &fn, &h->bk_emit_err)) fn = nullptr;
        h->bk_emit.push_back({K, fn});
        hit = &h->bk_emit.back();
    }
    h->bk_emit_last = hit->fn ? 1 : -1;
    return hit->fn;
}

static int bk_emit(void* fn, const shb_plan& B, const shb_out& O, const shb_cols& OC, sh_device_run* run,
                   hipStream_t stream) {
    return fn ? shb_emit_spec(fn, &B, &O, &OC, 0, run->d_out_seq, run->d_out_values, run->out_capacity, stream)
              : shb_emit(&B, &O, &OC, 0, run->d_out_seq, run->d_out_values, run->out_capacity, stream);
}

static constexpr int SH_BK_SEG_CHUNKS = 32;

static int bucket_launch(sh_handle* h, sh_device_run* run, shb_plan& B, const shb_out& O, const shb_cols& OC,
                         const shb_aggc* AG) {
    hipStream_t st = h->stream;
    void* args[] = {&B};
    void* const efn = bk_emit_fn(h, O, OC);
    int seg = SH_BK_SEG_CHUNKS;
    if (const char* e = getenv("SH_BK_SEG")) seg = atoi(e);
    if (seg > 0) seg = std::max(seg, (B.n_chunks + sh_handle::SH_BK_SEGS - 1) / sh_handle::SH_BK_SEGS);
    const int n_seg = seg > 0 ? (B.n_chunks + seg - 1) / seg : 1;
    const bool piped = !AG && !B.prof && (n_seg >= 2 || (seg > 0 && getenv("SH_BK_SEG")));
    if (piped && !h->bk_side) {
        if (hipStreamCreateWithFlags(&h->bk_side, hipStreamNonBlocking) != hipSuccess) {
            h->bk_side = nullptr;
            return fail(h, SH_E_HIP, "bucket side stream");
        }
    }
    for (auto& e : h->bk_ev)
        if (piped && !e && hipEventCreateWithFlags(&e, hipEventDisableTiming) != hipSuccess) {
            e = nullptr;
            return fail(h, SH_E_HIP, "bucket events");
        }
    if (piped) {
        hipStream_t sd = h->bk_side;
        auto quit = [&](const char* what) {
            hipStreamSynchronize(sd);
            hipStreamSynchronize(st);
            return fail(h, SH_E_HIP, what);
        };
        for (int k = 0; k < n_seg; k++) {
            const int c0 = k * seg, c1 = std::min(c0 + seg, B.n_chunks);
            B.c0 = c0;
            B.et0 = c0 * B.ct;
            B.et1 = std::min(c1 * B.ct, B.nt);
            if (hipModuleLaunchKernel((hipFunction_t)h->bk.match, (unsigned)(SHB_NB * (c1 - c0)), 1, 1, 512, 1, 1, 0, st,
                                      args, nullptr) != hipSuccess)
                return quit("shb_match launch failed");
            if (hipEventRecord(h->bk_ev[k], st) != hipSuccess || hipStreamWaitEvent(sd, h->bk_ev[k], 0) != hipSuccess)
                return quit("bucket segment event");
            if (shb_finish_seg(&B, B.et0, B.et1, B.ms_ctr + 2, k == n_seg - 1, sd)) return quit("bucket scan launch failed");
            if (bk_emit(efn, B, O, OC, run, sd))
                return quit("bucket emit launch failed");
        }
        hipEventRecord(h->ev[2], st);
        if (hipEventRecord(h->bk_ev[sh_handle::SH_BK_SEGS], sd) != hipSuccess ||
            hipStreamWaitEvent(st, h->bk_ev[sh_handle::SH_BK_SEGS], 0) != hipSuccess)
            return quit("bucket join event");
    } else {
        if (hipModuleLaunchKernel((hipFunction_t)h->bk.match, (unsigned)(SHB_NB * B.n_chunks), 1, 1, 512, 1, 1, 0, st,
                                  args, nullptr) != hipSuccess)
            return fail(h, SH_E_HIP, "shb_match launch failed");
        if (AG && shb_agg_carry(&B, AG, st)) return fail(h, SH_E_HIP, "aggregate carry launch failed");
        if (shb_finish(&B, h->w_scan.as<uint32_t>(), st)) return fail(h, SH_E_HIP, "bucket scan launch failed");
        hipEventRecord(h->ev[2], st);
        if (bk_emit(efn, B, O, OC, run, st)) return fail(h, SH_E_HIP, "bucket emit launch failed");
    }
    return SH_OK;
}

int run_bucket(sh_handle* h, sh_device_run* run, int32_t nkeys, BkAgg mode, BkRun* res) {
    static const bool off = getenv("SH_DISABLE_BUCKET") != nullptr;
    h->bk_last = 0;
    h->bk_emit_last = 0;
    *res = BkRun{};
    const shp_program& P = h->prog;
    const int64_t n = run->n;
    if (off || !h->partitioned || nkeys < 1024 || !P.out_fast || n < SHB_TILE) return 1;
    for (int o = 0; o < P.n_out; o++)
        if (P.out_agg[o] == SH_AGG_MAX || P.out_agg[o] == SH_AGG_MIN) return 1;
    const int kb = std::max(0, bits_for((uint64_t)(nkeys - 1)) - 8);
    if (kb > 8) return 1;
    shb_out O;
    shb_select S;
    if (shb_plan_select(P, h->part_attr0, run->d_cols, &O, &S)) return 1;
    if (h->bk_state == 0) {
        const int lrc = shj_bucket_load(&P, S.ms, S.n_ms, &h->bk, &h->bk_err);
        h->bk_state = lrc == 0 ? 1 : (lrc == -1 ? -2 : -1);
    }
    if (h->bk_state != 1) return 1;
    if (n >= ((int64_t)1 << 32) - SHB_TILE) return 1;
    shb_plan B{};
    B.n_staged = h->bk.n_staged;
    for (int k = 0; k < B.n_staged; k++) {
        B.st_src[k] = run->d_cols[h->bk.staged_attr[k]];
        B.st_width[k] = type_width(P.attr_type[0][h->bk.staged_attr[k]]);
    }
    shb_aggc AG{};
    int agg_of[SHB_MAX_OUT];
    bool carry = P.agg_post && mode != BK_AGG_ROWS;
    if (carry) {
        const shb_carry_plan cp = shb_plan_carry(P, run->d_cols, S.ms_of, &B, &AG, agg_of);
        if (cp == SHB_CARRY_NA) return 1;
        carry = cp == SHB_CARRY;
    }
    AG.parallel = mode == BK_AGG_PAR ? 1 : 0;
    if (P.agg_post && !carry && h->out_mode != SHB_OUT_RAW && !h->cols_rows) return 1;
    if (const int wrc = bk_workspace(h, run, kb, true, "bucket workspace", &B)) return wrc;
    static const int ct_env = getenv("SH_BK_CT") ? atoi(getenv("SH_BK_CT")) : 0;
    B.ct = ct_env > 0 ? std::min(ct_env, SHB_CT_MAX) : std::min(shj_bucket_chunk() * 15 / 512, SHB_CT_MAX);
    B.n_chunks = (B.nt + B.ct - 1) / B.ct;
    B.within = std::max<int64_t>(0, P.within_ms);
    for (int k = 0; k < B.n_staged; k++) {
        if (h->bk_st[k].ensure_fresh((int64_t)B.nt * SHB_TILE * B.st_width[k])) return fail(h, SH_E_OOM, "bucket workspace");
        B.st_dst[k] = h->bk_st[k].p;
    }
    B.n_ms = S.n_ms;
    const int64_t ms_vals = (int64_t)SHB_NB * B.n_chunks * SHB_SPAN + n;
    for (int m = 0; m < S.n_ms; m++) {
        B.ms_width[m] = type_width(P.attr_type[0][S.ms[m]]);
        if (h->bk_ms[m].ensure_fresh(ms_vals * B.ms_width[m])) return fail(h, SH_E_OOM, "match stream");
        B.ms[m] = h->bk_ms[m].p;
    }
    for (int i = 0; carry && i < AG.n; i++) {
        if (h->bk_agg[i].ensure_fresh(ms_vals * 8)) return fail(h, SH_E_OOM, "aggregate columns");
        AG.out[i] = h->bk_agg[i].p;
    }
    for (int o = 0; o < O.n_out; o++) {
        if (S.ms_of[o] >= 0) O.src[o] = B.ms[S.ms_of[o]];
        if (carry && agg_of[o] >= 0) {
            O.kind[o] = 0;
            O.src[o] = AG.out[agg_of[o]];
            O.type[o] = P.out_type[o];
        }
    }
    shb_cols OC{};
    if (!P.agg_post || carry) {
        int32_t wd[SHB_MAX_OUT];
        for (int o = 0; o < O.n_out; o++) wd[o] = type_width(O.type[o]);
        direct_layout(h, run, wd, O.n_out, &OC);
    }
    hipStream_t st = h->stream;
    hipMemcpyAsync(h->bk_rd.p, run->d_ts, 8, hipMemcpyDeviceToHost, st);
    if (hipStreamSynchronize(st) != hipSuccess) return fail(h, SH_E_HIP, "bucket: timestamp read");
    B.tbase = *h->bk_rd.as<int64_t>() - ((int64_t)1 << (31 - kb));
    if (const int brc = bk_begin(h, run, nkeys, &B, "bucket partition launch failed")) return brc;
    if (const int lrc = bucket_launch(h, run, B, O, OC, carry ? &AG : nullptr)) return lrc;
    int32_t flag = 0;
    int64_t total = 0;
    if (const int erc = bk_end(h, &B, "device error in bucket engine", &flag, &total)) return erc;
    if (B.prof) {
        unsigned long long pr[16];
        hipMemcpy(pr, B.prof, 128, hipMemcpyDeviceToHost);
        fprintf(stderr, "[shb_match clock ticks, sum over workgroups] table %llu load %llu rank %llu walk %llu "
                        "scan+psum %llu emit %llu\n",
                pr[5], pr[0], pr[1], pr[2], pr[3], pr[4]);
        if (carry && AG.parallel)
            fprintf(stderr, "[k_bk_aggp clock ticks, sum over workgroups] table+load %llu sort %llu rows %llu "
                            "scans %llu\n",
                    pr[8], pr[9], pr[10], pr[11]);
        else if (carry)
            fprintf(stderr, "[k_bk_aggc clock ticks, sum over workgroups] table %llu load+prefix %llu e1 %llu "
                            "sort %llu walk %llu\n",
                    pr[8], pr[9], pr[10], pr[11], pr[12]);
    }
    if (flag == SHB_F_AGG && carry && AG.parallel) {
        h->aggp_refused = res->refused = true;
        return 1;
    }
    const int rc = bk_close(h, run, flag, total, &h->bk_last, "bucket engine");
    if (h->bk_last && carry) {
        res->carried = mode;
        h->agg_last = AG.parallel ? 5 : 4;
    }
    return rc;
}

int run_s3b(sh_handle* h, sh_device_run* run, int32_t nkeys) {
    const bool off = getenv("SH_DISABLE_S3B") != nullptr || getenv("SH_NO_SEQ3") != nullptr;
    h->s3b_last = 0;
    h->bk_emit_last = 0;
    if (off || !h->partitioned || h->T->n_queries != 1 || !h->T->q[0].s3 || nkeys < 1024 || run->n < SHB_TILE)
        return 1;
    const nf_query& Q = h->T->q[0];
    const int kb = std::max(0, bits_for((uint64_t)(nkeys - 1)) - 8);
    if (kb > 12 || Q.contains_agg) return 1;
    const int A = Q.s3_a2, ty = Q.s3_t2;
    if (!(ty == SH_T_FLOAT || ty == SH_T_INT) || A < 0 || A >= (int)h->stream_types[0].size() ||
        type_width(h->stream_types[0][A]) != 4 || Q.s3_a3 != A || Q.s3_e1a != A || Q.s3_la != A || Q.s3_t3 != ty ||
        Q.s3_e1t != ty || Q.s3_lt != ty)
        return 1;
    shb_out O{};
    O.n_out = Q.n_out;
    shb_s3 S{};
    S.type = ty;
    S.warm = 1;
    S.op2 = Q.s3_op2;
    S.dom2 = Q.s3_dom2;
    S.op3 = Q.s3_op3;
    S.dom3 = Q.s3_dom3;
    int ms_of[SHB_MAX_OUT];
    for (int o = 0; o < Q.n_out; o++) {
        if (Q.s3_out_attr[o] != A || Q.s3_out_type[o] != ty) return 1;
        O.type[o] = ty;
        ms_of[o] = -1;
        const int sl = Q.s3_out_slot[o];
        if (sl == 2) {
            O.kind[o] = 1;
            O.src[o] = run->d_cols[A];
            continue;
        }
        int m = 0;
        while (m < S.n_ms && S.ms_slot[m] != sl) m++;
        if (m == S.n_ms) S.ms_slot[S.n_ms++] = sl;
        O.kind[o] = 0;
        ms_of[o] = m;
    }
    shb_plan B{};
    if (const int wrc = bk_workspace(h, run, kb, false, "sequence workspace", &B)) return wrc;
    const int64_t slots = (int64_t)B.nt * SHB_TILE;
    if (h->bk_st[0].ensure_fresh(slots * 4)) return fail(h, SH_E_OOM, "sequence workspace");
    B.n_staged = 1;
    B.st_src[0] = run->d_cols[A];
    B.st_dst[0] = h->bk_st[0].p;
    B.st_width[0] = 4;
    B.n_ms = S.n_ms;
    for (int m = 0; m < S.n_ms; m++) {
        if (h->bk_ms[m].ensure_fresh(slots * 4)) return fail(h, SH_E_OOM, "match stream");
        B.ms[m] = h->bk_ms[m].p;
        B.ms_width[m] = 4;
    }
    for (int o = 0; o < O.n_out; o++)
        if (ms_of[o] >= 0) O.src[o] = B.ms[ms_of[o]];
    shb_cols OC;
    int32_t wd[SHB_MAX_OUT];
    for (int o = 0; o < O.n_out; o++) wd[o] = 4;
    direct_layout(h, run, wd, O.n_out, &OC);
    hipStream_t st = h->stream;
    if (const int brc = bk_begin(h, run, nkeys, &B, "sequence partition failed")) return brc;
    if (shb_s3_carry(&B, &S, st)) return fail(h, SH_E_HIP, "sequence carry launch failed");
    if (shb_finish(&B, h->w_scan.as<uint32_t>(), st)) return fail(h, SH_E_HIP, "sequence scan failed");
    hipEventRecord(h->ev[2], st);
    if (bk_emit(bk_emit_fn(h, O, OC), B, O, OC, run, st)) return fail(h, SH_E_HIP, "sequence emit failed");
    int32_t flag = 0;
    int64_t total = 0;
    if (const int erc = bk_end(h, &B, "device error in the sequence engine", &flag, &total)) return erc;
    if (B.prof) {
        unsigned long long pr[16];
        hipMemcpy(pr, B.prof, 128, hipMemcpyDeviceToHost);
        fprintf(stderr, "[k_s3b clock ticks, sum over workgroups] tables+load %llu sort %llu carry %llu out %llu\n",
                pr[0], pr[1], pr[2], pr[3]);
    }
    return bk_close(h, run, flag, total, &h->s3b_last, "sequence engine");
}

int run_window(sh_handle* h, sh_device_run* run, int32_t nkeys) {
    if (h->stream_types[0].size() > 7) return 1;
    const shd_batch B = device_batch(h, run);
    int64_t nm = 0;
    const int64_t n = run->n;
    hipStream_t st = h->stream;
    if (ensure_ws(h, n)) return fail(h, SH_E_OOM, "workspace");
    const int na = (int)h->stream_types[0].size();
    const bool sorted = h->partitioned;
    shd_window_ws wws{};
    if (h->v_mpos.ensure_fresh(n * 4) || h->v_flag.ensure_fresh(64) || h->v_cnts.ensure_fresh(n * 4))
        return fail(h, SH_E_OOM, "window workspace");
    shd_payload carry;
    void* mid[8] = {nullptr};
    int alias = -1;
    if (sorted && carry_setup(h, run, &carry, mid, &alias)) return fail(h, SH_E_OOM, "window workspace");
    wws.match_pos = h->v_mpos.as<int32_t>();
    wws.cnt_s = h->v_cnts.as<uint32_t>();
    wws.cnt = h->w_cnt.as<uint32_t>();
    wws.off = h->w_off.as<uint32_t>();
    wws.flag = h->v_flag.as<int32_t>();
    const int tshift = sorted ? tile_shift_for(n, nkeys) : 0;
    hipEventRecord(h->ev[0], st);
    shd_segment_ws ws = seg_ws(h, n);
    const uint32_t* perm = nullptr;
    const uint32_t* skeys = nullptr;
    if (shd_segment_payload(&B, nkeys, &ws, st, &perm, &skeys, sorted ? &carry : nullptr, mid, tshift, 0))
        return fail(h, SH_E_HIP, "segment launch failed");
    shd_tiles TL{};
    if (tshift) {
        TL.K1 = (uint32_t)nkeys + 1;
        TL.ntile = (uint32_t)((n + ((int64_t)1 << tshift) - 1) >> tshift);
        TL.shift = tshift;
        const size_t words = (size_t)TL.ntile * TL.K1;
        if (h->v_dir.ensure_fresh(words * 8)) return fail(h, SH_E_OOM, "tile directory");
        TL.dstart = h->v_dir.as<uint32_t>();
        TL.dend = h->v_dir.as<uint32_t>() + words;
        if (shd_tile_dir(skeys, n, tshift, TL.K1, TL.ntile, (uint32_t*)TL.dstart, (uint32_t*)TL.dend, st))
            return fail(h, SH_E_HIP, "tile directory launch failed");
    }
    hipEventRecord(h->ev[1], st);
    const int64_t* sts = sorted ? h->v_sts.as<int64_t>() : run->d_ts;
    const void* scols[32];
    for (int a = 0; a < na; a++) scols[a] = sorted ? (const void*)h->v_scol[a].p : run->d_cols[a];
    if (alias >= 0) scols[alias] = skeys;
    if (h->jit_state == 0) {
        if (getenv("SH_DISABLE_JIT")) {
            h->jit_state = -1;
            h->jit_err = "disabled by SH_DISABLE_JIT";
        } else {
            h->jit_state = shj_window_load(&h->prog, &h->jit, &h->jit_err) == 0 ? 1 : -1;
        }
    }
    int wrc = shd_window(h->d_prog.as<shp_program>(), &h->prog, &B, nkeys, perm, skeys, sts, scols, &wws,
                         h->d_cols_desc.as<shd_cols>(), h->w_scan.as<uint32_t>(), run->d_out_seq, nullptr,
                         run->d_out_values, nullptr, run->out_capacity, &nm, st, h->ev[2],
                         h->jit_state == 1 ? &h->jit : nullptr, tshift ? &TL : nullptr);
    hipEventRecord(h->ev[3], st);
    if (hipStreamSynchronize(st) != hipSuccess) return fail(h, SH_E_HIP, "device error in window engine");
    if (wrc < 0) return fail(h, SH_E_HIP, "window engine launch failed");
    run->out_count = nm;
    if (wrc == 2) return fail(h, SH_E_MORE, "output capacity too small");
    if (wrc == 1) return 1;
    if (run->d_out_query && nm > 0) hipMemsetAsync(run->d_out_query, 0, nm * 4, st);
    phase_times(h);
    h->times.advance_launches = 1;
    return SH_OK;
// ... 60 lines not shown
```

### siddhi_amd/csrc/sh_host_int.h

```cpp
#pragma once

#include <hip/hip_runtime.h>

#include <algorithm>
#include <chrono>
#include <atomic>
#include <condition_variable>
#include <cstdio>
#include <cstdlib>
#include <cstring>
#include <deque>
#include <memory>
#include <mutex>
#include <string>
#include <thread>
#include <vector>

#include "../../include/siddhi_hip.h"
#include "sh_agg.h"
#include "sh_agg_seq.h"
#include "sh_bucket_plan.h"
#include "sh_device.h"
#include "sh_having.h"
#include "sh_jit.h"
#include "sh_jmap.h"
#include "sh_nfa.h"
#include "sh_rate.h"
#include "sh_nfa_dev.h"
#include "sh_nfa_lower.h"
#include "sh_rules.h"

namespace shh {

struct DevBuf {
    void* p = nullptr;
    size_t bytes = 0;
    bool view = false;
    void set_view(void* at, size_t n) {
        p = at;
        bytes = n;
        view = true;
    }
    int ensure(size_t need) {
        if (need <= bytes) return 0;
        if (view) return SH_E_OOM;
        size_t nb = std::max(need, bytes * 2);
        void* q = nullptr;
        if (hipMalloc(&q, nb) != hipSuccess) return SH_E_OOM;
        if (p) {
            hipMemcpy(q, p, bytes, hipMemcpyDeviceToDevice);
            hipFree(p);
        }
        p = q;
        bytes = nb;
        return 0;
    }
    int ensure_fresh(size_t need) {
        if (need <= bytes) return 0;
        if (view) return SH_E_OOM;
        if (p) hipFree(p);
        p = nullptr;
        bytes = 0;
        size_t nb = std::max(need, (size_t)4096);
        if (hipMalloc(&p, nb) != hipSuccess) return SH_E_OOM;
        bytes = nb;
        return 0;
    }
    void release() {
        if (p && !view) hipFree(p);
        p = nullptr;
        bytes = 0;
        view = false;
    }
    template <class T>
    T* as() const {
        return (T*)p;
    }
};

struct PinBuf {
    void* p = nullptr;
    size_t bytes = 0;
    int ensure(size_t need) {
        if (need <= bytes) return 0;
        release();
        size_t nb = std::max(need * 2, (size_t)1 << 16);
        if (hipHostMalloc(&p, nb, hipHostMallocDefault) != hipSuccess) {
            p = nullptr;
            return SH_E_OOM;
        }
        bytes = nb;
        return 0;
    }
    void release() {
        if (p) {
            hipDeviceSynchronize();
            hipHostFree(p);
        }
        p = nullptr;
        bytes = 0;
    }
    template <class T>
    T* as(size_t byte_off = 0) const {
// ... 161 lines not shown
    std::mutex hw_mu;
    std::deque<HistJob> hw_q;
    std::atomic<int> hw_pending{0};
    std::atomic<bool> hw_stop{false};
    std::condition_variable hw_cv;
    bool hw_spin = true;
    bool hw_fail = false;
    PinBuf pin_ctl2;
    hipEvent_t hw_ev[16] = {};
    int hw_ev_next = 0;
    double hw_ms = 0.0;
    bool hist_spec = false;
    std::vector<nfd_cand> pick_slots;
    PinBuf pin_sev, pin_rk, pin_cand;
    int64_t sev_cap = 0;
    int caps[6] = {16, 32, 64, 32, 8, 4};
    int32_t n_nkeys = 0;
    int64_t rec_cap = 0;
    int64_t clock = 0;
    uint64_t tick = 1;
    bool started = false;
    uint32_t batch_id = 0;
    bool has_rules = false;
    bool r_partitioned = false;
    int32_t r_nout = 0;
    std::vector<shr_rule> r_rules;
    bool r_aggp = false;
    int32_t r_agg[SHP_MAX_OUT] = {0}, r_argt[SHP_MAX_OUT] = {0};
    DevBuf a_q;
    std::vector<int64_t> r_ixval;
    std::vector<uint32_t> r_ixstart, r_ixrule, r_free;
    std::vector<int8_t> r_ixterm;
    shr_table r_tab{};
    DevBuf rd_rules, rd_ixval, rd_ixstart, rd_ixrule, rd_free, rd_tab;
    DevBuf rd_img;
    DevBuf r_tsr, v_ts32, v_sts32, v_mid_ts32;
    shr_img r_img{};
    DevBuf r_rec, r_keys, r_g, r_sk, r_sv, r_hist, r_scan, r_run;
    DevBuf rs_pr, rs_key, rs_list, rs_ctl, rs_live;
    int rs_last = 0;
    std::vector<int64_t> rq_ts;
    std::vector<int32_t> rq_key;
    std::vector<uint64_t> rq_seq;
    std::vector<uint32_t> rq_run;
    std::vector<uint8_t> rq_col[8];
    uint32_t rq_run_next = 0;
    bool rq_nullbit = false;
    uint64_t rq_call = 0, rq_call0 = 0;
    struct RuleStore {
        DevBuf ts, key, seq, run, col[8], c_off, c_rule;
    };
    RuleStore rc[2];
    int rc_cur = 0;
    int64_t rc_rows = 0, rc_pairs = 0;
    int64_t rc_steps = 0;
    DevBuf rc_klast;
    int32_t rc_nkeys = 0;
    DevBuf rc_ws, rc_oq, rc_ots;
    const uint64_t* step_seqs = nullptr;
    int64_t* step_ots = nullptr;
    int32_t* step_okey = nullptr;
    CarryTab ag_tab;
    DevBuf rc_okey;
    int bk_state = 0;
    int32_t part_attr0 = -1;
    int bk_last = 0;
    int s3b_last = 0;
    shj_bucket bk{};
    std::string bk_err;
    DevBuf bk_w0, bk_sp, bk_toff, bk_tofft, bk_tpfx, bk_tpfb, bk_cnt, bk_mstart, bk_tpre, bk_tfirst, bk_hstart, bk_ttot, bk_flag, bk_prof;
    DevBuf bk_st[SHB_MAX_STAGED], bk_ms[SHB_MAX_MS], bk_agg[SHB_MAX_AGG];
    PinBuf bk_rd;
    static constexpr int SH_BK_SEGS = 64;
    hipStream_t bk_side = nullptr;
    hipEvent_t bk_ev[SH_BK_SEGS + 1] = {};
    struct BkEmit {
        shj_emit_key key;
        void* fn;
    };
    std::vector<BkEmit> bk_emit;
    std::string bk_emit_err;
    int bk_emit_last = 0;
    bool aggp_refused = false;
    DevBuf w_colrows;
    bool cols_rows = false;
    int out_mode = SHB_OUT_RAW;
    int32_t pk_w[SHB_MAX_OUT], pk_woff[SHB_MAX_OUT], pk_rw = 0;
    DevBuf w_packseq;
    DevBuf a_scratch, a_seq;
    int agg_last = 0;
    bool hv_on = false;
    bool hv_chain = false;
    std::vector<shv_prog> hv_progs;
    DevBuf hv_d_progs;
    RowStage hv;
    bool rl_on = false;
    std::vector<shl_rule> rl_rules;
    DevBuf rl_d_rules;
    RowStage rl;
    CarryTab rl_tab;
    std::vector<int32_t> out_types;
    uint64_t fp = 0;
};

struct HpScope {
    sh_handle* h;
    int i;
    std::chrono::steady_clock::time_point t0;
    static bool on() {
        static const bool v = getenv("SH_HOST_PROF") != nullptr;
        return v;
    }
    HpScope(sh_handle* hh, int ii) : h(on() ? hh : nullptr), i(ii) {
        if (h) t0 = std::chrono::steady_clock::now();
    }
    ~HpScope() {
        if (!h) return;
        h->hp_ms[i] += std::chrono::duration<double, std::milli>(std::chrono::steady_clock::now() - t0).count();
        h->hp_n[i]++;
    }
};

void nf_hist_stop(sh_handle* h);

inline hipError_t nf_sync(sh_handle* h, hipStream_t st) {
    HpScope w_(h, 10);
    return hipStreamSynchronize(st);
}

int ensure_ws(sh_handle* h, int64_t n);
int fail(sh_handle* h, int code, const std::string& m);
int flush(sh_handle* h);
int nf_launch(sh_handle* h, NfLaunch& L);
int nf_complete(sh_handle* h, NfLaunch& L, int64_t* n_rows);
int nf_settle(sh_handle* h);
int nf_app_pull(sh_handle* h);
int nf_ensure_keys(sh_handle* h, int32_t nkeys);
int nf_next_due(sh_handle* h, int64_t* out);
struct NfOpts {
    bool fresh = false;
    int64_t batch_events = 0;
    bool seq3 = false;
    const sh_device_run* carry_run = nullptr;
    const uint32_t* gidx = nullptr;
    int64_t n_idx = 0;
};
bool nf_takes_seq3(const sh_handle* h);
int nf_process(sh_handle* h, const shd_batch& B, int32_t nkeys, const nf_cols& cols_in, uint64_t* d_seq,
               int64_t* d_vals, int64_t cap, int64_t* n_rows, const NfOpts& o = NfOpts());
int nf_push(sh_handle* h, const sh_batch* b, int64_t r0, const uint32_t* index = nullptr, int64_t call_n = 0,
            int64_t call_last = 0);
int nf_sev_flush(sh_handle* h);
int nf_start(sh_handle* h);
int nf_timers(sh_handle* h, int64_t now, bool wall = false);
int nf_upload_table(sh_handle* h);
int agg_post(sh_handle* h, sh_device_run* run, int32_t nkeys, const int32_t* d_query, int n_query,
             const int32_t* agg_kind, const int32_t* arg_type, int n_out);
int agg_carry_cols(const sh_handle* h);
shq_table carry_table(const CarryTab& C);
int carry_reserve(sh_handle* h, CarryTab& C, int64_t add, int n_cols);
int carry_dump(const CarryTab& C, std::vector<uint64_t>& keys, std::vector<int64_t>& state);
int carry_load(sh_handle* h, CarryTab& C, int n_cols, const uint64_t* keys, const int64_t* state, int64_t n);
int bits_for(uint64_t v);
int carry_setup(sh_handle* h, const sh_device_run* run, shd_payload* carry, void** mid, int* alias,
                bool used_only = false, bool with_ts = true);
int rows_for_cols(sh_handle* h, sh_device_run* run);
void direct_layout(sh_handle* h, sh_device_run* run, const int32_t* widths, int n_out, shb_cols* OC);
shd_batch device_batch(const sh_handle* h, const sh_device_run* run);
void phase_times(sh_handle* h);
enum BkAgg { BK_AGG_ROWS = 0, BK_AGG_PAR, BK_AGG_SEQ };
struct BkRun {
    BkAgg carried = BK_AGG_ROWS;
    bool refused = false;
};
int run_bucket(sh_handle* h, sh_device_run* run, int32_t nkeys, BkAgg mode, BkRun* res);
int run_window(sh_handle* h, sh_device_run* run, int32_t nkeys);
int run_rules(sh_handle* h, sh_device_run* run);
int rules_stage(sh_handle* h, const sh_batch* b);
int rules_step(sh_handle* h);
int having_filter(sh_handle* h, int64_t m, int n_out, const shw_rows& src, const shw_rows_out& dst);
int rate_limit(sh_handle* h, int64_t m, int n_out, const shw_rows& src, const int32_t* keys, int32_t n_keys,
               const shq_table* T, const shw_rows_out& dst, const uint64_t** put_keys, const int64_t** put_state);
struct RowPost {
    bool step = false;
    shw_rows src{};
    int64_t m = 0;
    int n_out = 1;
    const shw_rows_out* end = nullptr;
    RowStage* mid = nullptr;
    size_t room = 0;
    const int32_t* d_keys = nullptr;
    int32_t n_keys = 1;
    CarryTab* tab = nullptr;
    int64_t after_having = 0, after_rate = 0;
    shw_rows out{};
    const uint64_t* put_keys = nullptr;
    const int64_t* put_state = nullptr;
};
int row_post(sh_handle* h, RowPost& P);
int run_s3b(sh_handle* h, sh_device_run* run, int32_t nkeys);
shd_segment_ws seg_ws(sh_handle* h, int64_t n);
int tile_shift_for(int64_t n, int32_t nkeys);

extern "C" {
int shx_jit_status(sh_handle* h);
int shx_jit_compile(sh_handle* h);
int shx_bucket_status(sh_handle* h);
int shx_seq3_status(sh_handle* h);
int shx_agg_status(sh_handle* h);
int shx_having_status(sh_handle* h);
int shx_having_rows(sh_handle* h, int64_t* rows_in, int64_t* rows_kept);
double shx_having_ms(sh_handle* h);
int shx_rate_status(sh_handle* h);
int shx_rate_rows(sh_handle* h, int64_t* rows_in, int64_t* rows_kept);
double shx_rate_ms(sh_handle* h);
uint64_t shx_fingerprint(sh_handle* h);
int shx_rules_status(sh_handle* h);
int shx_rules_carry(sh_handle* h, int64_t* partials, int64_t* rows);
int shx_rules_agg_carry(sh_handle* h, int64_t* entries);
int64_t shx_rules_agg_capacity(sh_handle* h);
int shx_host_profile(sh_handle* h, double* ms, int64_t* n, int cap);
int shx_seq3_shape(sh_handle* h);
int shx_bucket_compile(sh_handle* h, char* buf, int64_t len);
int shx_bucket_emit_status(sh_handle* h);
int shx_emit_compile(sh_handle* h, int layout, char* buf, int64_t len);
int shx_emit_compile_key(const int32_t* key, char* buf, int64_t len, char* err, int64_t err_len);
int64_t shx_jit_source(sh_handle* h, char* buf, int64_t len);
}
```

### siddhi_amd/csrc/sh_jit.cpp

```cpp
#include <hip/hip_runtime.h>
#include <hip/hiprtc.h>

#include <stdio.h>
#include <stdlib.h>
#include <string.h>

#include <algorithm>
#include <map>
#include <mutex>
#include <set>
#include <string>
#include <vector>

#include "../../include/sh_query.h"
#include "sh_device.h"
#include "sh_jit.h"
#include "sh_jit_src.inc"

namespace {

int type_width(int t) { return t == SH_T_LONG || t == SH_T_DOUBLE ? 8 : (t == SH_T_BOOL ? 1 : 4); }

int env_int(const char* name, int def, int lo, int hi) {
    const char* e = getenv(name);
// ... 875 lines not shown
             "    if (u == 0) flg_ |= (live & same & (wv[u] > tmono_ ? 1u : 0u)) ? (uint32_t)SHB_F_MONO : 0u;\n"
             "    const uint32_t act = live & same & (wv[u] >= tlo ? 1u : 0u);\n";
        for (int a : need_r)
            s += "    x0_" + std::to_string(a) + " = " + raw_of(P.attr_type[0][a], "av" + std::to_string(a) + "[u]") + ";\n";
        s += "    {\n" + cand_f +
             "    const uint32_t cons = act & (ok ? 1u : 0u);\n"
             "    call_ += cons;\n"
             "    mask |= cons << (step < SHB_MSTEPS ? step : SHB_MSTEPS);\n    }\n";
        s += "    {\n" + mid_f + "    }\n    live = act & (cmp_op<" + DT + ">(" + (mx ? std::to_string(SH_OP_GE)
                                                                                  : std::to_string(SH_OP_LE)) +
             ", Mx, xq) ? 0u : 1u);\n}\ntmono_ = ~0u;\nbase += SHB_D;\npp -= SHB_D;\n"
             "}\n"
             "if (__ballot(flg_ != 0u) != 0ull) {\n"
             "    const uint32_t f_ = (__ballot((flg_ & SHB_F_HALO) != 0u) ? (uint32_t)SHB_F_HALO : 0u) |\n"
             "                        (__ballot((flg_ & SHB_F_COUNT) != 0u) ? (uint32_t)SHB_F_COUNT : 0u) |\n"
             "                        (__ballot((flg_ & SHB_F_MONO) != 0u) ? (uint32_t)SHB_F_MONO : 0u);\n"
             "    if (dl_ == 0) atomicOr(P.flag, (int)f_);\n"
             "}\n}\n";
        return s;
    };
    auto walk = [&](bool count, const std::string& on_consumed) {
        return head() + slow(count, on_consumed, "sp - 1");
    };
    std::string ms_put;
    for (size_t m = 0; m < ms_attrs.size(); m++) {
        const int a = ms_attrs[m];
        ms_put += "        ((" + std::string(col_ctype(P.attr_type[0][a])) + "*)P.ms[" + std::to_string(m) +
                  "])[dst] = " + lds(a) + "[o];\n";
    }
    (void)sidx;
    const bool prof = shj_bucket_profiled() != 0;
    auto phase = [&](int ph) { return prof ? "SHB_PROF(" + std::to_string(ph) + ")\n" : std::string(); };

    src = SHJ_HEADERS;
    const int64_t wlim = P.within_ms < 0 ? 0 : (P.within_ms > 0xFFFFFFFFll ? 0xFFFFFFFFll : P.within_ms);
    src += "\n#define SHJ_W " + lit64(P.within_ms) + "\n#define SHB_WLIM " + std::to_string(wlim) +
           "u\n#define SHB_TPB 512\n#define SHB_D " + std::to_string(kWalkBlock) +
           "\n#define SHB_MOVF 0x8000u\n#define SHB_MSTEPS 15\nstatic_assert(SHB_MOVF == 1u << SHB_MSTEPS, \"mask\");\n"
           "#define SHB_MINB " + std::to_string(kMatchMinBlocks) + "\n"
           "#define SHB_NSEG (SHB_CT_MAX + SHB_HMAX)\n"
           "#define SHB_SPANJ " + std::to_string(kSpan) + "\n#define SHB_CHJ " + std::to_string(kChunk) + "\n" +
           "#define SHB_NR (SHB_SPANJ / SHB_TPB)\nstatic_assert(SHB_SPANJ % SHB_TPB == 0 && SHB_NR * SHB_TPB == SHB_SPANJ && SHB_SPANJ <= SHB_SPAN && SHB_CHJ <= SHB_CH && SHB_CHJ % SHB_TPB == 0, \"span\");\n"
           "static_assert(SHB_NSEG < 256 && SHB_NSEG < SHB_TPB, \"segments\");\n";
    src += R"(
extern "C" __global__ void __launch_bounds__(SHB_TPB, SHB_MINB) shb_match(shb_plan P) {
__shared__ uint32_t s_ws[SHB_SPANJ];
// the chunk's consumers in sorted order: sorted position | (arrival - hl) << 16
__shared__ uint32_t s_cons[SHB_CHJ];
__shared__ uint16_t s_pre[SHB_CHJ];
__shared__ uint32_t u_buf[(SHB_TPB / 64) * 256];  // rank phase: per-wave key counts; then the u16 consumed masks
uint32_t (*const wcnt)[256] = (uint32_t(*)[256])u_buf;
uint16_t* const s_msk = (uint16_t*)u_buf;
static_assert((SHB_TPB / 64) * 256 * 4 >= SHB_CHJ * 2, "masks fit u_buf");
// run: halo events per local key, then their inclusive prefix over the keys
__shared__ uint32_t run[256], tstart[256], ws[SHB_TPB / 64];
// the workgroup's segment table, loaded once: per tile of [A - SHB_HMAX, E] the
// bucket's events in the tiles before it (the partition's prefix, P.tpfx + P.tpfb)
// and per tile of [A - SHB_HMAX, E) the global index of its segment's first
// event; per chunk tile the halo start (k_bk_prep_a: tile a - 1 and the tiles
// before it that the window can reach). A pass's segments are a slice of the
// table (seg_p, seg_g below); seg_of[j]: segment of span event 32 j
__shared__ uint32_t tb_p[SHB_NSEG + 1];
__shared__ uint32_t tb_g[SHB_NSEG];
__shared__ int32_t tb_h[SHB_CT_MAX];
// the latest timestamp before each table tile (k_bk_prep_b's tpre): with it in the
// one load, a pass waits for no global load before its span's
__shared__ int64_t tb_t[SHB_NSEG];
__shared__ uint8_t seg_of[SHB_SPANJ / 32];
__shared__ int s_i[2];
)";
    for (int a : staged_out)
        src += "__shared__ " + std::string(col_ctype(P.attr_type[0][a])) + " " + lds(a) + "[SHB_SPANJ];\n";
    for (size_t k = 0; k < staged_out.size(); k++) {
        const int a = staged_out[k];
        const std::string ct = col_ctype(P.attr_type[0][a]);
        src += "const " + ct + "* __restrict__ g_a" + std::to_string(a) + " = (const " + ct + "*)P.st_dst[" +
               std::to_string(k) + "];\n";
    }
    src += R"(
// consecutive buckets on one XCD (blocks are dealt round-robin to the 8 XCDs):
// neighbouring segments of a tile share cache lines
// (the launch holds the chunks from P.c0 on: every global quantity goes by the chunk's
// index in the step, none by the grid; SHB_NB is a multiple of 8, so the XCD of a
// block is that of its position in the launch)
const uint32_t gbid = (uint32_t)P.c0 * SHB_NB + blockIdx.x;
const int b = (int)((gbid & 7u) * (SHB_NB / 8) + ((gbid >> 3) & (SHB_NB / 8 - 1)));
const int A = (int)(gbid / SHB_NB) * P.ct;
const int E = A + P.ct < P.nt ? A + P.ct : P.nt;
const int kb = P.kb;
const uint32_t kmask = (1u << kb) - 1u;
const int lane = (int)(threadIdx.x & 63u), wv = (int)(threadIdx.x >> 6);
)";
    if (prof) src += "unsigned long long t_prev = wall_clock64();  // (the table load counts with the first pass's table phase)\n";
    src += R"(const int T0 = A - SHB_HMAX;  // the table's first tile (entries of tiles < 0 are never read)
{
    const int Tm = T0 + (int)threadIdx.x;
    if (Tm >= 0 && Tm <= E) {
        // (tile tstride, one past the last block: the bucket's total alone)
        const uint32_t in = Tm < P.tstride ? P.tpfx[(int64_t)b * P.tstride + Tm] : 0u;
        tb_p[threadIdx.x] = in + P.tpfb[(int64_t)b * (P.tstride / 64 + 1) + (Tm >> 6)];
        if (Tm < E) {
            tb_g[threadIdx.x] = ((uint32_t)Tm << SHB_TILE_SHIFT) + P.tofft[(int64_t)b * P.tstride + Tm];
            tb_t[threadIdx.x] = P.tpre[Tm];
        }
    }
    if (A + (int)threadIdx.x < E) tb_h[threadIdx.x] = P.hstart[A + (int)threadIdx.x];
}
for (int a = A; a < E;) {
__syncthreads();
)";
    if (prof)
        src += "if (a != A) t_prev = wall_clock64();\n"
               "#define SHB_PROF(ph) if (P.prof && threadIdx.x == 0) { const unsigned long long t_now = wall_clock64(); "
               "atomicAdd(&P.prof[ph], t_now - t_prev); t_prev = t_now; }\n";
    src += R"(// the pass's segments, one per tile from the first halo tile h0: seg_p[t] the
// events of the bucket before segment t (only differences are used), seg_g[t] the
// global index of its first event
const int h0 = tb_h[a - A];
const int nseg = E - h0;
const uint32_t* const seg_p = tb_p + (h0 - T0);
const uint32_t* const seg_g = tb_g + (h0 - T0);
// this pass: consumers from tiles [a, a + ne), at most SHB_CHJ events; the halo
// from segment sb on (trimmed at the front when it and tile a overflow the span)
const int ta = a - h0;
const uint32_t pa = seg_p[ta];
// (both counts by every wave for itself, over the at most SHB_HMAX halo and
// SHB_CT_MAX chunk segments: the table is read-only here, so no barrier)
int sb = 0, ne = 0;
for (int x = lane; x - lane < ta; x += 64)
    sb += (int)__popcll(__ballot(x < ta && seg_p[ta + 1] - seg_p[x] > SHB_SPANJ));
const uint32_t sbase = seg_p[sb];
for (int x = ta + lane; x - lane < nseg; x += 64)
    ne += (int)__popcll(__ballot(x < nseg && seg_p[x + 1] - pa <= SHB_CHJ && seg_p[x + 1] - sbase <= SHB_SPANJ));
if (ne == 0) {
    // tile a's segment alone exceeds a chunk
    if (threadIdx.x == 0) atomicOr(P.flag, SHB_F_SPAN);
    a++;
    continue;
}
const int se = ta + ne;      // one past the pass's last segment
const int hs = h0 + sb;      // the span's first tile (> 0: earlier events exist)
const int L = (int)(seg_p[se] - sbase), hl = (int)(pa - sbase), nc = L - hl;
// a walk that leaves its key's run in the span while still in the window could
// have missed earlier events of the key only if some event before the span is
// as late as the window's start (tpre: the latest timestamp before each tile)
const int64_t tmx_ = hs > 0 ? tb_t[hs - T0] - P.tbase : INT64_MIN;
#define SHB_OFF(t32) ((int64_t)(t32) - SHJ_W <= tmx_)
// seg_of by the segments themselves: a segment owns the 32-event blocks whose
// first event lies in it (the last segment starting at or before that event;
// an empty segment owns none)
for (int t = sb + (int)threadIdx.x; t < se; t += SHB_TPB) {
    const uint32_t x1 = seg_p[t + 1] - sbase;
    for (uint32_t j = (seg_p[t] - sbase + 31u) >> 5; j * 32u < x1; j++) seg_of[j] = (uint8_t)t;
}
__syncthreads();
)";
    src += phase(5);
    src += R"(// global index of span event i (segments in span order)
#define SHB_GIDX(i, out) { int sg_ = seg_of[(i) >> 5]; while (seg_p[sg_ + 1] - sbase <= (uint32_t)(i)) sg_++; \
    out = seg_g[sg_] + ((uint32_t)(i) - (seg_p[sg_] - sbase)); }
if (threadIdx.x < 256) run[threadIdx.x] = 0u;
// the span into registers (all loads in flight together): wave v owns the
// contiguous span events [v * SHB_NR * 64, (v + 1) * SHB_NR * 64)
uint32_t wr[SHB_NR];
)";
    for (int a : staged_out)
        src += std::string(col_ctype(P.attr_type[0][a])) + " vr" + std::to_string(a) + "[SHB_NR];\n";
    src += R"(#pragma unroll
for (int k = 0; k < SHB_NR; k++) {
    const int i = (wv * SHB_NR + k) * 64 + lane;
    uint32_t gi = 0u;
    if (i < L) SHB_GIDX(i, gi)
    wr[k] = i < L ? P.w0[gi] : 0u;
)";
    for (int a : staged_out)
        src += "    vr" + std::to_string(a) + "[k] = i < L ? g_a" + std::to_string(a) + "[gi] : 0;\n";
    src += R"(}
for (int c = (int)threadIdx.x; c < (SHB_TPB / 64) * 256; c += SHB_TPB) (&wcnt[0][0])[c] = 0u;
__syncthreads();
)";
    src += phase(0);
    src += R"(// stable sort of the span by local key, staged in sorted order (the walks read
// consecutive LDS words): each wave ranks its own events (kb ballots per round,
// running per-key counts of the wave), one block pass combines the waves
uint32_t rw[SHB_NR];
{
    const uint64_t lt = lane ? (~0ull >> (64 - lane)) : 0ull;
#pragma unroll
    for (int k = 0; k < SHB_NR; k++) {
        const int i = (wv * SHB_NR + k) * 64 + lane;
        const bool valid = i < L;
        const uint32_t d = wr[k] & kmask;
        uint64_t peers = __ballot(valid);
#pragma unroll
        for (int bb = 0; bb < 8; bb++) {
            if (bb < kb) {  // uniform: the local key has kb bits
                const bool bit = (d >> bb) & 1u;
                const uint64_t m = __ballot(valid && bit);
                peers &= bit ? m : ~m;
            }
        }
// ... 431 lines not shown
```

### siddhi_amd/csrc/sh_vm.h

```cpp
#pragma once
#include <hip/hip_runtime.h>

#include "../../include/sh_query.h"
#include "sh_device.h"

struct VmVal {
    int64_t b;
    uint8_t t;
    uint8_t null;
};

__device__ __forceinline__ float bits_f32(int64_t b) { return __int_as_float((int32_t)(uint32_t)b); }
__device__ __forceinline__ double bits_f64(int64_t b) { return __longlong_as_double(b); }
__device__ __forceinline__ int64_t f32_bits(float f) { return (int64_t)(uint32_t)__float_as_int(f); }
__device__ __forceinline__ int64_t f64_bits(double d) { return __double_as_longlong(d); }

__device__ __forceinline__ int64_t to_i64(const VmVal& v) {
    return v.t == SH_T_LONG ? v.b : (int64_t)(int32_t)v.b;
}
__device__ __forceinline__ float to_f32(const VmVal& v) {
    switch (v.t) {
        case SH_T_INT: return (float)(int32_t)v.b;
        case SH_T_LONG: return (float)v.b;
        case SH_T_FLOAT: return bits_f32(v.b);
        default: return (float)bits_f64(v.b);
    }
}
__device__ __forceinline__ double to_f64(const VmVal& v) {
    switch (v.t) {
        case SH_T_INT: return (double)(int32_t)v.b;
        case SH_T_LONG: return (double)v.b;
        case SH_T_FLOAT: return (double)bits_f32(v.b);
        default: return bits_f64(v.b);
    }
}

template <typename T>
__device__ __forceinline__ bool cmp_op(int op, T a, T b) {
    switch (op) {
        case SH_OP_EQ: return a == b;
        case SH_OP_NE: return a != b;
        case SH_OP_GT: return a > b;
        case SH_OP_GE: return a >= b;
        case SH_OP_LT: return a < b;
        default: return a <= b;
    }
}


__device__ __forceinline__ bool vm_cmp(int op, int dom, const VmVal& l, const VmVal& r) {
    switch (dom) {
        case DOM_I32: return cmp_op<int32_t>(op, (int32_t)l.b, (int32_t)r.b);
        case DOM_I64: return cmp_op<int64_t>(op, to_i64(l), to_i64(r));
        case DOM_F32: return cmp_op<float>(op, to_f32(l), to_f32(r));
        case DOM_F64: return cmp_op<double>(op, to_f64(l), to_f64(r));
        case DOM_BOOL: return cmp_op<int>(op, l.b != 0, r.b != 0);
        default: return cmp_op<int32_t>(op, (int32_t)l.b, (int32_t)r.b);
    }
}

__device__ __forceinline__ VmVal vm_arith(int aop, int rt, const VmVal& l, const VmVal& r) {
    VmVal o;
    o.t = (uint8_t)rt;
    o.null = 0;
    o.b = 0;
    if (l.null || r.null) {
        o.null = 1;
    } else if (rt == SH_T_INT) {
        const uint32_t a = (uint32_t)l.b, b = (uint32_t)r.b;
        const int32_t sa = (int32_t)a, sb = (int32_t)b;
        int32_t res = 0;
        switch (aop) {
            case SH_OP_ADD: res = (int32_t)(a + b); break;
            case SH_OP_SUB: res = (int32_t)(a - b); break;
            case SH_OP_MUL: res = (int32_t)(a * b); break;
            case SH_OP_DIV:
                if (sb == 0) o.null = 1;
                else res = (sa == INT32_MIN && sb == -1) ? INT32_MIN : sa / sb;
                break;
            default:
                if (sb == 0) o.null = 1;
                else res = (sb == -1) ? 0 : sa % sb;
        }
        o.b = res;
    } else if (rt == SH_T_LONG) {
        const uint64_t a = (uint64_t)to_i64(l), b = (uint64_t)to_i64(r);
        const int64_t sa = (int64_t)a, sb = (int64_t)b;
        int64_t res = 0;
        switch (aop) {
            case SH_OP_ADD: res = (int64_t)(a + b); break;
            case SH_OP_SUB: res = (int64_t)(a - b); break;
            case SH_OP_MUL: res = (int64_t)(a * b); break;
            case SH_OP_DIV:
                if (sb == 0) o.null = 1;
                else res = (sa == INT64_MIN && sb == -1) ? INT64_MIN : sa / sb;
                break;
            default:
                if (sb == 0) o.null = 1;
                else res = (sb == -1) ? 0 : sa % sb;
        }
        o.b = res;
    } else if (rt == SH_T_FLOAT) {
        const float a = to_f32(l), b = to_f32(r);
        float res = 0.f;
        switch (aop) {
            case SH_OP_ADD: res = __fadd_rn(a, b); break;
            case SH_OP_SUB: res = __fsub_rn(a, b); break;
            case SH_OP_MUL: res = __fmul_rn(a, b); break;
            case SH_OP_DIV:
                if (b == 0.0f) o.null = 1;
                else res = __fdiv_rn(a, b);
                break;
            default:
                if (b == 0.0f) o.null = 1;
                else res = fmodf(a, b);
        }
        o.b = f32_bits(res);
    } else {
        const double a = to_f64(l), b = to_f64(r);
        double res = 0.0;
        switch (aop) {
            case SH_OP_ADD: res = __dadd_rn(a, b); break;
            case SH_OP_SUB: res = __dsub_rn(a, b); break;
            case SH_OP_MUL: res = __dmul_rn(a, b); break;
            case SH_OP_DIV:
                if (b == 0.0) o.null = 1;
                else res = __ddiv_rn(a, b);
                break;
            default:
                if (b == 0.0) o.null = 1;
                else res = fmod(a, b);
        }
        o.b = f64_bits(res);
    }
    return o;
}

__device__ __forceinline__ int64_t load_attr(const shd_cols* C, int s, int a, int type, uint32_t row) {
    const void* p = C->col[s][a];
    switch (type) {
        case SH_T_LONG: return ((const int64_t*)p)[row];
        case SH_T_FLOAT: return (int64_t)(uint32_t)((const uint32_t*)p)[row];
// ... 254 lines not shown
```

### siddhi_amd/device_run.py

```python
from __future__ import annotations

import ctypes as C

import numpy as np
import torch

from . import abi
from . import compiler as cp
from ._native import CompiledHandle, check, lib


_TORCH = {cp.LONG: torch.int64, cp.DOUBLE: torch.float64, cp.INT: torch.int32, cp.STRING: torch.int32,
          cp.FLOAT: torch.float32, cp.BOOL: torch.uint8}


def columns_to_raw(cols, types):
    out = np.empty((len(cols[0]) if cols else 0, len(cols)), dtype=np.int64)
    for o, (c, t) in enumerate(zip(cols, types)):
        if t == cp.FLOAT:
            out[:, o] = c.view(np.uint32).astype(np.int64)
        elif t == cp.DOUBLE:
            out[:, o] = c.view(np.int64)
        else:
            out[:, o] = c.astype(np.int64)
# ... 46 lines not shown
            if packed:
                if getattr(self, "_row_cap", 0) < cap or getattr(self, "_row_bytes", 0) != rb:
                    self.out_rows = torch.empty(cap * rb, dtype=torch.uint8, device=self.device)
                    self._row_cap, self._row_bytes = cap, rb
                if not hasattr(self, "out_q") or self.out_q.numel() < cap:
                    self.out_q = torch.empty(cap, dtype=torch.int32, device=self.device)
                r = abi.sh_device_run()
                r.version = abi.SH_DEVICE_RUN_V2
                r.out_layout = abi.SH_OUT_PACKED
                r.d_run = run_ids.data_ptr() if run_ids is not None else None
                r.n = n
                r.d_ts = ts.data_ptr()
                r.d_keys = keys.data_ptr()
                r.n_keys = int(n_keys)
                r.batch_events = int(batch_events)
                r.d_cols = (C.c_void_p * len(cols))(*[c.data_ptr() for c in cols])
                r.out_capacity = self._row_cap
                r.d_out_seq = None
                r.d_out_values = self.out_rows.data_ptr()
                r.stream = stream.cuda_stream if stream is not None else torch.cuda.current_stream(self.device).cuda_stream
                r.d_out_query = self.out_q.data_ptr() if with_query else None
                rc = lib().sh_run_device_v2(self.handle.h, C.byref(r))
                if rc == abi.SH_E_MORE and attempt == 0 and int(r.out_count) > self._row_cap:
                    cap = int(r.out_count)
                    continue
                check(self.handle.h, rc)
                m = int(r.out_count)
                res = (m, self.out_rows[: m * rb].view(m, rb))
                return res + (self.out_q[:m],) if with_query else res
            if self._out_cap < cap:
                self.out_seq = torch.empty(cap, dtype=torch.int64, device=self.device)
                self.out_vals = (torch.empty(0, dtype=torch.int64, device=self.device) if columns else
                                 torch.empty(cap * self.n_out, dtype=torch.int64, device=self.device))
                self.out_q = torch.empty(cap, dtype=torch.int32, device=self.device)
                self._out_cap = cap
            if columns and (self._col_cap < self._out_cap or not hasattr(self, "out_cols")):
                self.out_cols = [torch.empty(self._out_cap, dtype=_TORCH[t], device=self.device)
                                 for t in self.out_types]
                self._col_cap = self._out_cap
            if not columns and self.out_vals.numel() < self._out_cap * self.n_out:
                self.out_vals = torch.empty(self._out_cap * self.n_out, dtype=torch.int64, device=self.device)
            cp = (C.c_void_p * len(cols))(*[c.data_ptr() for c in cols])
            r = abi.sh_device_run()
            r.version = abi.SH_DEVICE_RUN_V2
            r.d_run = run_ids.data_ptr() if run_ids is not None else None
            r.n = n
            r.d_ts = ts.data_ptr()
            r.d_keys = keys.data_ptr()
            r.n_keys = int(n_keys)
            r.batch_events = int(batch_events)
            r.d_cols = cp
            r.out_capacity = self._out_cap
            r.d_out_seq = self.out_seq.data_ptr()
            r.d_out_values = None if columns else self.out_vals.data_ptr()
            if columns:
                ocp = (C.c_void_p * len(self.out_cols))(*[c.data_ptr() for c in self.out_cols])
                r.d_out_cols = ocp
            r.stream = stream.cuda_stream if stream is not None else torch.cuda.current_stream(self.device).cuda_stream
            r.d_out_query = self.out_q.data_ptr() if with_query else None
            rc = lib().sh_run_device_v2(self.handle.h, C.byref(r))
            if rc == abi.SH_E_MORE and attempt == 0 and int(r.out_count) > self._out_cap:
                cap = int(r.out_count)
                continue
            check(self.handle.h, rc)
            break
        m = int(r.out_count)
        if columns:
            res = (m, self.out_seq[:m], [c[:m] for c in self.out_cols])
            return res + (self.out_q[:m],) if with_query else res
        res = (m, self.out_seq[:m], self.out_vals[: m * self.n_out].view(m, self.n_out))
        return res + (self.out_q[:m],) if with_query else res

    def kernel_times(self):
        t = abi.sh_kernel_times()
        lib().sh_last_kernel_times(self.handle.h, C.byref(t))
        return dict(segment_ms=t.segment_ms, advance_ms=t.advance_ms, emit_ms=t.emit_ms, total_ms=t.total_ms)

    def jit_status(self):
        return lib().shx_jit_status(self.handle.h)

    def bucket_status(self):
        return lib().shx_bucket_status(self.handle.h)

    def bucket_emit_status(self):
        return lib().shx_bucket_emit_status(self.handle.h)

    def seq3_status(self):
        return lib().shx_seq3_status(self.handle.h)

    def rules_status(self):
        return lib().shx_rules_status(self.handle.h)

    def agg_status(self):
        return lib().shx_agg_status(self.handle.h)

    def having_status(self):
        return lib().shx_having_status(self.handle.h)

    def having_rows(self):
        a, b = C.c_int64(0), C.c_int64(0)
        lib().shx_having_rows(self.handle.h, C.byref(a), C.byref(b))
        return a.value, b.value

    def having_ms(self):
        return lib().shx_having_ms(self.handle.h)

    def rate_status(self):
        return lib().shx_rate_status(self.handle.h)

    def rate_rows(self):
        a, b = C.c_int64(0), C.c_int64(0)
        lib().shx_rate_rows(self.handle.h, C.byref(a), C.byref(b))
        return a.value, b.value

    def rate_ms(self):
        return lib().shx_rate_ms(self.handle.h)

    def last_error(self):
        return lib().sh_last_error(self.handle.h).decode()

    def close(self):
        self.handle.close()
```

Measured before the change: 29.25 billion.

## Drop inert events in bucket scatter and cut chunks by valid-event counts

The bucket scatter kernel now evaluates the pattern's open and take filter predicates on staged columns and marks events that can satisfy neither as inert, so they are excluded from bucket placement. A new chunk table, built in the prep kernel from per-tile valid counts, cuts chunks by event volume instead of a fixed tile count, so downstream NFA passes process fewer and denser chunks. Ordering and span violations are detected with flags, and the host falls back to the non-drop path when timestamp or key order does not hold. The cost is extra column reads and predicate evaluation in scatter, an extra prep stage, and more complex halo bounds.

```diff
diff --git a/siddhi_amd/abi.py b/siddhi_amd/abi.py
--- a/siddhi_amd/abi.py
+++ b/siddhi_amd/abi.py
@@ -165,6 +165,8 @@
     lib.shx_bucket_compile.restype = C.c_int
     lib.shx_bucket_status.argtypes = [C.c_void_p]
     lib.shx_bucket_status.restype = C.c_int
+    lib.shx_bucket_drop_status.argtypes = [C.c_void_p]
+    lib.shx_bucket_drop_status.restype = C.c_int
     lib.shx_bucket_emit_status.argtypes = [C.c_void_p]
     lib.shx_bucket_emit_status.restype = C.c_int
     lib.shx_emit_compile.argtypes = [C.c_void_p, C.c_int, C.c_char_p, C.c_int64]
diff --git a/siddhi_amd/build.py b/siddhi_amd/build.py
--- a/siddhi_amd/build.py
+++ b/siddhi_amd/build.py
@@ -7,7 +7,7 @@
 OUT = os.path.join(HERE, "libsiddhi_hip.so")
 SOURCES = ["sh_host.cpp", "sh_host_nfa.cpp", "sh_host_fast.cpp", "sh_host_snap.cpp", "sh_jit.cpp", "sh_nfa_lower.cpp", "sh_kernels.hip", "sh_window.hip", "sh_nfa.hip", "sh_rules.hip", "sh_bucket.hip", "sh_shard.hip", "sh_agg.hip", "sh_having.hip", "sh_rate.hip"]
 JIT_HEADERS = [os.path.join(HERE, "..", "include", "sh_query.h"), os.path.join(CSRC, "sh_program.h"),
-               os.path.join(CSRC, "sh_device.h"), os.path.join(CSRC, "sh_vm.h"),
+               os.path.join(CSRC, "sh_device.h"), os.path.join(CSRC, "sh_cmp.h"), os.path.join(CSRC, "sh_vm.h"),
                os.path.join(CSRC, "sh_wave.h")]
 JIT_EMIT_HEADERS = [os.path.join(CSRC, "sh_rows.h"), os.path.join(CSRC, "sh_bk_emit.h")]
 JIT_INC = os.path.join(CSRC, "sh_jit_src.inc")
diff --git a/siddhi_amd/csrc/sh_bk_emit.h b/siddhi_amd/csrc/sh_bk_emit.h
--- a/siddhi_amd/csrc/sh_bk_emit.h
+++ b/siddhi_amd/csrc/sh_bk_emit.h
@@ -129,7 +129,8 @@
 #pragma unroll
         for (int j = 0; j < BK_ITEMS; j++) {
             const int l = l0 + j * 64;
-            sl[j] = l < tile_n ? (uint32_t)P.sp[b0 + l] : BK_NOSLOT;
+            const uint32_t s = l < tile_n ? (uint32_t)P.sp[b0 + l] : 0xFFFFu;
+            sl[j] = s != 0xFFFFu ? s : BK_NOSLOT;
         }
     }
     {
diff --git a/siddhi_amd/csrc/sh_bucket.hip b/siddhi_amd/csrc/sh_bucket.hip
--- a/siddhi_amd/csrc/sh_bucket.hip
+++ b/siddhi_amd/csrc/sh_bucket.hip
@@ -5,6 +5,7 @@
 #include "../../include/sh_query.h"
 #include "sh_device.h"
 #include "sh_nfa.h"
+#include "sh_bucket_drop.h"
 #include "sh_bk_emit.h"
 #include "sh_rows.h"
 #include "sh_wave.h"
@@ -12,10 +13,13 @@
 static inline unsigned bk_grid(int nt) { return 8u * (unsigned)((nt + 7) >> 3); }
 
 
-template <int MINW, int TPB>
-__global__ void __launch_bounds__(TPB, MINW) k_bk_scatter(const int32_t* __restrict__ keys,
-                                                          const int64_t* __restrict__ ts, int32_t nkeys, shb_plan P) {
+template <int MINW, int TPB, bool DROP>
+__global__ void __launch_bounds__(TPB, DROP ? 8 : MINW) k_bk_scatter(const int32_t* __restrict__ keys,
+                                                          const int64_t* __restrict__ ts, int32_t nkeys, shb_plan P,
+                                                          shi_pred D) {
     constexpr int SC_ITEMS = SHB_TILE / TPB;
+    __shared__ uint32_t s_d0[TPB / 64], s_dl[TPB / 64];
+    __shared__ uint32_t s_in[256];
     __shared__ uint32_t wcnt[TPB / 64][256];
     __shared__ uint32_t tstart[256];
     __shared__ uint32_t ws[TPB / 64];
@@ -25,7 +29,47 @@
     if (T < 0) return;
     const int64_t b0 = (int64_t)T << SHB_TILE_SHIFT;
     const int lane = threadIdx.x & 63, w = threadIdx.x >> 6;
+    uint32_t inert = 0u;
+    if constexpr (DROP) {
+        const int64_t e0 = b0 + (int64_t)w * (64 * SC_ITEMS) + lane;
+        uint32_t ok_o = ~0u, ok_t = ~0u;
+#pragma unroll 1
+        for (int q = 0; q < D.n_open + D.n_take; q++) {
+            const shi_term tm = q < D.n_open ? D.open[q] : D.take[q - D.n_open];
+            const uint32_t* __restrict__ src = (const uint32_t*)P.st_src[tm.col];
+            uint32_t m = 0u;
+            if (tm.width == 8) {
+#pragma unroll
+                for (int hf = 0; hf < 2; hf++) {
+                    uint2 v[SC_ITEMS / 2];
+#pragma unroll
+                    for (int j = 0; j < SC_ITEMS / 2; j++) {
+                        const int64_t i = e0 + (hf * (SC_ITEMS / 2) + j) * 64;
+                        v[j] = i < P.n ? ((const uint2*)src)[i] : make_uint2(0u, 0u);
+                    }
+#pragma unroll
+                    for (int j = 0; j < SC_ITEMS / 2; j++)
+                        m |= (shi_term_ok(tm, (int64_t)(((uint64_t)v[j].y << 32) | v[j].x)) ? 1u : 0u)
+                             << (hf * (SC_ITEMS / 2) + j);
+                }
+            } else {
+                uint32_t v[SC_ITEMS];
+#pragma unroll
+                for (int j = 0; j < SC_ITEMS; j++) {
+                    const int64_t i = e0 + j * 64;
+                    v[j] = i < P.n ? src[i] : 0u;
+                }
+#pragma unroll
+                for (int j = 0; j < SC_ITEMS; j++) m |= (shi_term_ok(tm, (int64_t)v[j]) ? 1u : 0u) << j;
+            }
+            if (q < D.n_open) ok_o &= m;
+            else ok_t &= m;
+        }
+        inert = ~(ok_o | ok_t);
+    }
     for (int c = threadIdx.x; c < (TPB / 64) * 256; c += TPB) (&wcnt[0][0])[c] = 0u;
+    if constexpr (DROP)
+        if (threadIdx.x < 256) s_in[threadIdx.x] = 0u;
     __syncthreads();
     int32_t key[SC_ITEMS];
     uint32_t rw[SC_ITEMS], wp[SC_ITEMS];
@@ -72,6 +116,28 @@
         if (lane == 0) s_tmx[w] = tmx;
         if (threadIdx.x == 0) P.tfirst[T] = tv[0];
     }
+    if constexpr (DROP) {
+        const int64_t e0 = b0 + (int64_t)w * (64 * SC_ITEMS) + lane;
+        bool viol = false;
+        uint32_t dl = 0u;
+#pragma unroll
+        for (int j = 0; j < SC_ITEMS; j++) {
+            const uint32_t d = wp[j] >> P.kb;
+            uint32_t p = (uint32_t)__shfl_up((int)d, 1);
+            if (lane == 0) p = j ? dl : d;
+            viol |= e0 + j * 64 < P.n && (key[j] < 0 || p > d);
+            dl = (uint32_t)__shfl((int)d, 63);
+            if (j == 0 && lane == 0) s_d0[w] = d;
+        }
+        if (lane == 0) s_dl[w] = dl;
+        if (viol) atomicOr(P.flag, SHB_F_ORDER);
+#pragma unroll
+        for (int j = 0; j < SC_ITEMS; j++)
+            if (inert >> j & 1u) {
+                if (rw[j] != ~0u) atomicAdd(&s_in[rw[j] >> 16], 1u);
+                rw[j] = ~0u;
+            }
+    }
     {
         uint32_t old[SC_ITEMS];
 #pragma unroll
@@ -98,6 +164,10 @@
         }
     }
     __syncthreads();
+    if constexpr (DROP) {
+        if (lane == 0 && w > 0 && b0 + (int64_t)w * (64 * SC_ITEMS) < P.n && s_dl[w - 1] > s_d0[w])
+            atomicOr(P.flag, SHB_F_ORDER);
+    }
     uint32_t nvalid;
     {
         uint32_t tot = 0;
@@ -109,6 +179,8 @@
                 tot += c;
             }
         }
+        if constexpr (DROP)
+            if (threadIdx.x < 256 && tot + s_in[threadIdx.x] > (uint32_t)P.span_lim) atomicOr(P.flag, SHB_F_SPAN);
         const uint32_t ex = shw_block_excl<TPB>(threadIdx.x < 256 ? tot : 0u, ws, &nvalid);
         if (threadIdx.x < 256) {
             tstart[threadIdx.x] = ex;
@@ -179,16 +251,17 @@
 
 
 __device__ __forceinline__ void bk_halo(const int64_t* __restrict__ tfirst, int32_t* __restrict__ hstart, int32_t nt,
-                                        int64_t within, int t) {
+                                        int64_t within, int t, int hcap) {
     if (t >= nt) return;
     const int64_t ta = tfirst[t];
     const int64_t tlim = ta < INT64_MIN + within ? INT64_MIN : ta - within;
     int h = t > 0 ? 1 : 0;
-    while (h < t && h < SHB_HMAX && tfirst[t - h] >= tlim) h++;
+    while (h < t && h < hcap && tfirst[t - h] >= tlim) h++;
     hstart[t] = t - h;
 }
 
-__device__ __forceinline__ void bk_tpre(int64_t* __restrict__ tpre, int32_t nt, int64_t* s) {
+__device__ __forceinline__ void bk_tpre(int64_t* __restrict__ tpre, int32_t nt, int64_t* s,
+                                        const int64_t* __restrict__ tfirst, int32_t* __restrict__ flag) {
     const int per = (nt + 1023) / 1024;
     const int t0 = threadIdx.x * per;
     int64_t m = INT64_MIN;
@@ -205,7 +278,58 @@
     for (int t = t0; t < t0 + per && t < nt; t++) {
         const int64_t v = tpre[t];
         tpre[t] = run;
+        if (tfirst && run > tfirst[t]) atomicOr(flag, SHB_F_ORDER);
         run = v > run ? v : run;
+    }
+}
+
+#define BK_CUT_TILES 8192
+__device__ __forceinline__ void bk_cut(const uint16_t* __restrict__ toff, int32_t nt, int32_t* __restrict__ ctab,
+                                       int k, int seg_tiles, int slots, int ct, int cut, int32_t* __restrict__ flag,
+                                       uint32_t* pfx, uint16_t* nxt, uint32_t* ws) {
+    const int t0 = k * seg_tiles, S = nt - t0 < seg_tiles ? nt - t0 : seg_tiles;
+    int32_t* __restrict__ tab = ctab + 2 * (int64_t)k * slots;
+    if (!cut) {
+        for (int j = threadIdx.x; j < slots; j += 1024) {
+            const int a = j * ct < S ? j * ct : S, e = a + ct < S ? a + ct : S;
+            tab[2 * j] = t0 + a;
+            tab[2 * j + 1] = t0 + e;
+        }
+        return;
+    }
+    constexpr int PER = BK_CUT_TILES / 1024;
+    uint32_t v[PER], sum = 0;
+#pragma unroll
+    for (int q = 0; q < PER; q++) {
+        const int i = (int)threadIdx.x * PER + q;
+        v[q] = i < S ? (uint32_t)toff[(int64_t)(t0 + i) * SHB_TOFF + 256] : 0u;
+        sum += v[q];
+    }
+    uint32_t tot;
+    uint32_t off = shw_block_excl<1024>(sum, ws, &tot);
+    if (threadIdx.x == 0) pfx[0] = 0u;
+#pragma unroll
+    for (int q = 0; q < PER; q++) {
+        off += v[q];
+        pfx[threadIdx.x * PER + q + 1] = off;
+    }
+    __syncthreads();
+#pragma unroll
+    for (int q = 0; q < PER; q++) {
+        const int i = (int)threadIdx.x * PER + q;
+        if (i < S) nxt[i] = (uint16_t)shb_cut_next(pfx, i, S, (uint32_t)ct << SHB_TILE_SHIFT, SHB_CT_MAX);
+    }
+    __syncthreads();
+    if (threadIdx.x == 0) {
+        int a = 0, j = 0;
+        for (; a < S && j < slots; j++) {
+            const int e = nxt[a];
+            tab[2 * j] = t0 + a;
+            tab[2 * j + 1] = t0 + e;
+            a = e;
+        }
+        if (a < S) atomicOr(flag, SHB_F_SPAN);
+        for (; j < slots; j++) tab[2 * j] = tab[2 * j + 1] = t0 + S;
     }
 }
 
@@ -974,10 +1098,10 @@
                                                     uint16_t* __restrict__ tofft, int stride,
                                                     uint32_t* __restrict__ tpfx, uint32_t* __restrict__ tpfb, int nbt,
                                                     const int64_t* __restrict__ tfirst, int32_t* __restrict__ hstart,
-                                                    int64_t within) {
+                                                    int64_t within, int hcap) {
     __shared__ uint16_t s[TT_T][SHB_NB + 2];
     if ((int)blockIdx.x >= nbt) {
-        bk_halo(tfirst, hstart, nt, within, ((int)blockIdx.x - nbt) * 1024 + (int)threadIdx.x);
+        bk_halo(tfirst, hstart, nt, within, ((int)blockIdx.x - nbt) * 1024 + (int)threadIdx.x, hcap);
         return;
     }
     const int T0 = (int)blockIdx.x * TT_T;
@@ -1000,14 +1124,22 @@
     }
 }
 
-__global__ void __launch_bounds__(1024) k_bk_prep_b(uint32_t* __restrict__ tpfb, int nbt, int64_t* __restrict__ tpre,
-                                                    int32_t nt, int ntp) {
+__global__ void __launch_bounds__(1024) k_bk_prep_b(uint32_t* __restrict__ tpfb, int nbt, int ntp, int ncut, int order,
+                                                    shb_plan P) {
     __shared__ int64_t s[1024];
+    __shared__ uint32_t c_pfx[BK_CUT_TILES + 1], c_ws[1024 / 64];
+    __shared__ uint16_t c_nxt[BK_CUT_TILES];
     if ((int)blockIdx.x < ntp) {
-        bk_tpre(tpre, nt, s);
+        bk_tpre(P.tpre, P.nt, s, order ? P.tfirst : nullptr, P.flag);
         return;
     }
-    const int b = ((int)blockIdx.x - ntp) * (1024 / 64) + (int)(threadIdx.x >> 6), lane = (int)(threadIdx.x & 63u);
+    if ((int)blockIdx.x < ntp + ncut) {
+        bk_cut(P.toff, P.nt, P.ctab, (int)blockIdx.x - ntp, P.seg_tiles, P.seg_slots, P.ct, P.cut, P.flag, c_pfx, c_nxt,
+               c_ws);
+        return;
+    }
+    if (!tpfb) return;
+    const int b = ((int)blockIdx.x - ntp - ncut) * (1024 / 64) + (int)(threadIdx.x >> 6), lane = (int)(threadIdx.x & 63u);
     if (b >= SHB_NB) return;
     uint32_t* row = tpfb + (int64_t)b * (nbt + 1);
     uint32_t carry = 0;
@@ -1020,20 +1152,30 @@
     }
 }
 
-extern "C" int shb_partition(const int32_t* keys, const int64_t* ts, int32_t nkeys, shb_plan* P, void* stream) {
+extern "C" int shb_partition(const int32_t* keys, const int64_t* ts, int32_t nkeys, shb_plan* P, const void* drop,
+                             void* stream) {
     hipStream_t st = (hipStream_t)stream;
-    hipLaunchKernelGGL((k_bk_scatter<2, 1024>), dim3(bk_grid(P->nt)), dim3(1024), 0, st, keys, ts, nkeys, *P);
+    const shi_pred* D = (const shi_pred*)drop;
+    const bool dropping = D && D->on;
+    if (dropping && (P->no_ts || !P->ctab)) return -1;
+    if (P->ctab && (P->n_seg < 1 || P->seg_slots < 1 || (P->cut && P->seg_tiles > BK_CUT_TILES))) return -1;
+    if (dropping)
+        hipLaunchKernelGGL((k_bk_scatter<2, 1024, true>), dim3(bk_grid(P->nt)), dim3(1024), 0, st, keys, ts, nkeys, *P, *D);
+    else
+        hipLaunchKernelGGL((k_bk_scatter<2, 1024, false>), dim3(bk_grid(P->nt)), dim3(1024), 0, st, keys, ts, nkeys, *P,
+                           shi_pred{});
     if (bk_ok()) return -3;
     if (P->tstride < P->nt) return -1;
-    const int nbt = (P->nt + TT_T - 1) / TT_T, ntp = P->no_ts ? 0 : 1;
+    const int nbt = (P->nt + TT_T - 1) / TT_T, ntp = P->no_ts ? 0 : 1, ncut = P->ctab ? P->n_seg : 0;
     const bool pfx = P->tpfx && P->tpfb;
     if (pfx && P->tstride != nbt * TT_T) return -1;
     hipLaunchKernelGGL(k_bk_prep_a, dim3(nbt + (P->no_ts ? 0 : (P->nt + 1023) / 1024)), dim3(1024), 0, st,
                        (const uint16_t*)P->toff, P->nt, P->tofft, P->tstride, pfx ? P->tpfx : nullptr,
-                       pfx ? P->tpfb : nullptr, nbt, P->tfirst, P->hstart, P->within);
-    if (ntp || pfx)
-        hipLaunchKernelGGL(k_bk_prep_b, dim3(ntp + (pfx ? SHB_NB / (1024 / 64) : 0)), dim3(1024), 0, st, P->tpfb, nbt,
-                           P->tpre, P->nt, ntp);
+                       pfx ? P->tpfb : nullptr, nbt, P->tfirst, P->hstart, P->within,
+                       P->cut ? SHB_HMAX + SHB_CT_MAX : SHB_HMAX);
+    if (ntp || pfx || ncut)
+        hipLaunchKernelGGL(k_bk_prep_b, dim3(ntp + ncut + (pfx ? SHB_NB / (1024 / 64) : 0)), dim3(1024), 0, st,
+                           pfx ? P->tpfb : nullptr, nbt, ntp, ncut, dropping ? 1 : 0, *P);
     return bk_ok();
 }
 
diff --git a/siddhi_amd/csrc/sh_bucket_drop.h b/siddhi_amd/csrc/sh_bucket_drop.h
--- /dev/null
+++ b/siddhi_amd/csrc/sh_bucket_drop.h
@@ -0,0 +1,140 @@
+#pragma once
+#include <stdint.h>
+
+#include "sh_cmp.h"
+
+#define SHI_MAX_TERMS 2
+
+struct shi_term {
+    int32_t col, width, type;
+    int32_t op, dom, ctype;
+    int64_t c;
+};
+
+struct shi_pred {
+    int32_t on;
+    int32_t n_open, n_take;
+    int32_t pad;
+    shi_term open[SHI_MAX_TERMS], take[SHI_MAX_TERMS];
+};
+
+SHV_HD bool shi_term_ok(const shi_term& T, int64_t bits) {
+    VmVal l, r;
+    l.b = bits;
+    l.t = (uint8_t)T.type;
+    l.null = 0;
+    r.b = T.c;
+    r.t = (uint8_t)T.ctype;
+    r.null = 0;
+    return vm_cmp(T.op, T.dom, l, r);
+}
+
+SHV_HD int shb_cut_next(const uint32_t* pfx, int a, int S, uint32_t cap, int tmax) {
+    int lo = a + 1, hi = a + tmax < S ? a + tmax : S;
+    while (lo < hi) {
+        const int mid = (lo + hi + 1) >> 1;
+        if (pfx[mid] - pfx[a] <= cap) lo = mid;
+        else hi = mid - 1;
+    }
+    return lo;
+}
+
+SHV_HD int shb_cut_bound(int S, int ct) {
+    if (S <= 0) return 0;
+    if (ct < 2) return S;
+    const int k = (S - 1) / (ct - 1) + 1;
+    return k < S ? k : S;
+}
+
+#if !defined(__HIPCC_RTC__)
+namespace shi {
+inline bool numeric_dom(int d) { return d == DOM_I32 || d == DOM_I64 || d == DOM_F32 || d == DOM_F64; }
+inline bool numeric_type(int t) { return t == SH_T_INT || t == SH_T_LONG || t == SH_T_FLOAT || t == SH_T_DOUBLE; }
+inline bool ordering(int op) { return op == SH_OP_GT || op == SH_OP_GE || op == SH_OP_LT || op == SH_OP_LE; }
+inline bool upward(int op) { return op == SH_OP_GT || op == SH_OP_GE; }
+inline int mirror(int op) {
+    switch (op) {
+        case SH_OP_GT: return SH_OP_LT;
+        case SH_OP_GE: return SH_OP_LE;
+        case SH_OP_LT: return SH_OP_GT;
+        case SH_OP_LE: return SH_OP_GE;
+        default: return op;
+    }
+}
+inline bool unary(const shp_term& T, int attr_type, shi_term* o) {
+    if (T.rkind != 1 || !numeric_dom(T.dom) || !numeric_type(attr_type) || !numeric_type(T.ctype)) return false;
+    o->col = T.lattr;
+    o->type = attr_type;
+    o->width = (attr_type == SH_T_LONG || attr_type == SH_T_DOUBLE) ? 8 : 4;
+    o->op = T.op;
+    o->dom = T.dom;
+    o->ctype = T.ctype;
+    o->c = T.c;
+    return true;
+}
+}
+
+inline void shi_derive(const shp_program& P, shi_pred* D) {
+    *D = shi_pred{};
+    if (!P.window_ok) return;
+    for (int k = 0; k < 2; k++)
+        if (!P.filter_fast[k] && P.filter_pc[k] >= 0) return;
+    shi_pred R{};
+    auto push = [&](shi_term* side, int32_t* n, const shi_term& t) {
+        if (*n == SHI_MAX_TERMS) return false;
+        side[(*n)++] = t;
+        return true;
+    };
+    const int nf1 = P.filter_fast[0] ? P.filter_nterms[0] : 0;
+    const int nf2 = P.filter_fast[1] ? P.filter_nterms[1] : 0;
+    shi_term t;
+    for (int k = 0; k < nf1; k++) {
+        const shp_term& T = P.terms[0][k];
+        if (T.lslot != 0 || !shi::unary(T, P.attr_type[0][T.lattr], &t) || !push(R.open, &R.n_open, t)) return;
+    }
+    const shp_term* cross = nullptr;
+    for (int k = 0; k < nf2; k++) {
+        const shp_term& T = P.terms[1][k];
+        if (T.rkind == 1 || T.lslot == T.rslot) {
+            if (!shi::unary(T, P.attr_type[0][T.lattr], &t)) return;
+            if (!(T.lslot ? push(R.take, &R.n_take, t) : push(R.open, &R.n_open, t))) return;
+            continue;
+        }
+        if (cross) return;
+        cross = &T;
+    }
+    if (cross && cross->rkind == 0 && shi::ordering(cross->op) && shi::numeric_dom(cross->dom)) {
+        const bool q_left = cross->lslot == 1;
+        const int op = q_left ? cross->op : shi::mirror(cross->op);
+        const int xa = q_left ? cross->lattr : cross->rattr, ya = q_left ? cross->rattr : cross->lattr;
+        const int xt = P.attr_type[0][xa];
+        for (int k = 0; k < nf1 && shi::numeric_type(xt); k++) {
+            const shp_term& F = P.terms[0][k];
+            if (F.rkind != 1 || F.lattr != ya || F.dom != cross->dom || !shi::ordering(F.op) ||
+                shi::upward(F.op) != shi::upward(op) || !shi::numeric_type(F.ctype))
+                continue;
+            const bool eq = (op == SH_OP_GE || op == SH_OP_LE) && (F.op == SH_OP_GE || F.op == SH_OP_LE);
+            t.col = xa;
+            t.type = xt;
+            t.width = (xt == SH_T_LONG || xt == SH_T_DOUBLE) ? 8 : 4;
+            t.op = shi::upward(op) ? (eq ? SH_OP_GE : SH_OP_GT) : (eq ? SH_OP_LE : SH_OP_LT);
+            t.dom = cross->dom;
+            t.ctype = F.ctype;
+            t.c = F.c;
+            if (!push(R.take, &R.n_take, t)) return;
+            break;
+        }
+    }
+    if (R.n_open == 0 || R.n_take == 0) return;
+    R.on = 1;
+    *D = R;
+}
+
+inline bool shi_inert(const shi_pred& D, const int64_t* attr_bits) {
+    if (!D.on) return false;
+    bool open = true, take = true;
+    for (int k = 0; k < D.n_open; k++) open = open && shi_term_ok(D.open[k], attr_bits[D.open[k].col]);
+    for (int k = 0; k < D.n_take; k++) take = take && shi_term_ok(D.take[k], attr_bits[D.take[k].col]);
+    return !open && !take;
+}
+#endif
diff --git a/siddhi_amd/csrc/sh_cmp.h b/siddhi_amd/csrc/sh_cmp.h
--- /dev/null
+++ b/siddhi_amd/csrc/sh_cmp.h
@@ -0,0 +1,67 @@
+#pragma once
+#include <stdint.h>
+
+#include "../../include/sh_query.h"
+#include "sh_program.h"
+
+#if defined(__HIPCC_RTC__)
+#define SHV_HD __device__ __forceinline__
+#elif defined(__HIPCC__) || defined(__HIP__)
+#define SHV_HD __host__ __device__ __forceinline__
+#else
+#define SHV_HD inline
+#endif
+
+struct VmVal {
+    int64_t b;
+    uint8_t t;
+    uint8_t null;
+};
+
+SHV_HD float bits_f32(int64_t b) { return __builtin_bit_cast(float, (uint32_t)b); }
+SHV_HD double bits_f64(int64_t b) { return __builtin_bit_cast(double, b); }
+SHV_HD int64_t f32_bits(float f) { return (int64_t)__builtin_bit_cast(uint32_t, f); }
+SHV_HD int64_t f64_bits(double d) { return __builtin_bit_cast(int64_t, d); }
+
+SHV_HD int64_t to_i64(const VmVal& v) {
+    return v.t == SH_T_LONG ? v.b : (int64_t)(int32_t)v.b;
+}
+SHV_HD float to_f32(const VmVal& v) {
+    switch (v.t) {
+        case SH_T_INT: return (float)(int32_t)v.b;
+        case SH_T_LONG: return (float)v.b;
+        case SH_T_FLOAT: return bits_f32(v.b);
+        default: return (float)bits_f64(v.b);
+    }
+}
+SHV_HD double to_f64(const VmVal& v) {
+    switch (v.t) {
+        case SH_T_INT: return (double)(int32_t)v.b;
+        case SH_T_LONG: return (double)v.b;
+        case SH_T_FLOAT: return (double)bits_f32(v.b);
+        default: return bits_f64(v.b);
+    }
+}
+
+template <typename T>
+SHV_HD bool cmp_op(int op, T a, T b) {
+    switch (op) {
+        case SH_OP_EQ: return a == b;
+        case SH_OP_NE: return a != b;
+        case SH_OP_GT: return a > b;
+        case SH_OP_GE: return a >= b;
+        case SH_OP_LT: return a < b;
+        default: return a <= b;
+    }
+}
+
+SHV_HD bool vm_cmp(int op, int dom, const VmVal& l, const VmVal& r) {
+    switch (dom) {
+        case DOM_I32: return cmp_op<int32_t>(op, (int32_t)l.b, (int32_t)r.b);
+        case DOM_I64: return cmp_op<int64_t>(op, to_i64(l), to_i64(r));
+        case DOM_F32: return cmp_op<float>(op, to_f32(l), to_f32(r));
+        case DOM_F64: return cmp_op<double>(op, to_f64(l), to_f64(r));
+        case DOM_BOOL: return cmp_op<int>(op, l.b != 0, r.b != 0);
+        default: return cmp_op<int32_t>(op, (int32_t)l.b, (int32_t)r.b);
+    }
+}
diff --git a/siddhi_amd/csrc/sh_device.h b/siddhi_amd/csrc/sh_device.h
--- a/siddhi_amd/csrc/sh_device.h
+++ b/siddhi_amd/csrc/sh_device.h
@@ -83,6 +83,7 @@
 #define SHB_F_COUNT 8
 #define SHB_F_HALO 16
 #define SHB_F_SPAN 32
+#define SHB_F_ORDER 128
 
 struct shb_plan {
     int64_t n;
@@ -108,7 +109,10 @@
     int32_t tstride;
     int32_t c0;
     int32_t et0, et1;
-    int32_t pad_t;
+    int32_t cut;
+    int32_t* ctab;
+    int32_t n_seg, seg_tiles, seg_slots;
+    int32_t span_lim;
     uint32_t* tpfx;
     uint32_t* tpfb;
     uint8_t* cnt;
@@ -191,7 +195,7 @@
                    uint32_t* const* vbuf, uint32_t* hist, uint32_t* scan_tmp, void* stream,
                    const uint32_t** keys_out, const uint32_t** vals_out);
 int shd_exclusive_scan(const uint32_t* in, uint32_t* out, int64_t n, uint32_t* tmp, void* stream);
-int shb_partition(const int32_t* keys, const int64_t* ts, int32_t nkeys, shb_plan* P, void* stream);
+int shb_partition(const int32_t* keys, const int64_t* ts, int32_t nkeys, shb_plan* P, const void* drop, void* stream);
 int shb_finish(shb_plan* P, uint32_t* scan_tmp, void* stream);
 int shb_finish_seg(shb_plan* P, int32_t t0, int32_t t1, uint32_t* carry, int last, void* stream);
 int shb_s3_carry(const shb_plan* P, const shb_s3* S, void* stream);
diff --git a/siddhi_amd/csrc/sh_host.cpp b/siddhi_amd/csrc/sh_host.cpp
--- a/siddhi_amd/csrc/sh_host.cpp
+++ b/siddhi_amd/csrc/sh_host.cpp
@@ -1712,6 +1712,8 @@
     return h->bk_last;
 }
 
+int shx_bucket_drop_status(sh_handle* h) { return h ? h->drop_last : 0; }
+
 int shx_bucket_emit_status(sh_handle* h) {
     if (!h) return 0;
     if (h->bk_emit_last < 0) h->err = h->bk_emit_err;
diff --git a/siddhi_amd/csrc/sh_host_fast.cpp b/siddhi_amd/csrc/sh_host_fast.cpp
--- a/siddhi_amd/csrc/sh_host_fast.cpp
+++ b/siddhi_amd/csrc/sh_host_fast.cpp
@@ -1004,12 +1004,13 @@
     return SH_OK;
 }
 
-static int bk_begin(sh_handle* h, const sh_device_run* run, int32_t nkeys, shb_plan* B, const char* what) {
+static int bk_begin(sh_handle* h, const sh_device_run* run, int32_t nkeys, shb_plan* B, const shi_pred* drop,
+                    const char* what) {
     hipStream_t st = h->stream;
     hipEventRecord(h->ev[0], st);
     hipMemsetAsync(B->flag, 0, 32, st);
     hipMemsetAsync(B->ttot, 0, ((int64_t)B->nt + 1) * 4, st);
-    if (shb_partition(run->d_keys, run->d_ts, nkeys, B, st)) return fail(h, SH_E_HIP, what);
+    if (shb_partition(run->d_keys, run->d_ts, nkeys, B, drop, st)) return fail(h, SH_E_HIP, what);
     hipEventRecord(h->ev[1], st);
     return SH_OK;
 }
@@ -1065,16 +1066,26 @@
 
 static constexpr int SH_BK_SEG_CHUNKS = 32;
 
+static bool bk_segments(shb_plan& B, bool carry) {
+    const int n_nom = (B.nt + B.ct - 1) / B.ct;
+    int seg = SH_BK_SEG_CHUNKS;
+    if (const char* e = getenv("SH_BK_SEG")) seg = atoi(e);
+    if (seg > 0) seg = std::max(seg, (n_nom + sh_handle::SH_BK_SEGS - 1) / sh_handle::SH_BK_SEGS);
+    const int n_seg = seg > 0 ? (n_nom + seg - 1) / seg : 1;
+    const bool piped = !carry && !B.prof && (n_seg >= 2 || (seg > 0 && getenv("SH_BK_SEG")));
+    B.n_seg = piped ? n_seg : 1;
+    B.seg_tiles = piped ? seg * B.ct : B.nt;
+    return piped;
+}
+
+static int bk_seg_slots(const shb_plan& B, int S) { return B.cut ? shb_cut_bound(S, B.ct) : (S + B.ct - 1) / B.ct; }
+
 static int bucket_launch(sh_handle* h, sh_device_run* run, shb_plan& B, const shb_out& O, const shb_cols& OC,
-                         const shb_aggc* AG) {
+                         const shb_aggc* AG, bool piped) {
     hipStream_t st = h->stream;
     void* args[] = {&B};
     void* const efn = bk_emit_fn(h, O, OC);
-    int seg = SH_BK_SEG_CHUNKS;
-    if (const char* e = getenv("SH_BK_SEG")) seg = atoi(e);
-    if (seg > 0) seg = std::max(seg, (B.n_chunks + sh_handle::SH_BK_SEGS - 1) / sh_handle::SH_BK_SEGS);
-    const int n_seg = seg > 0 ? (B.n_chunks + seg - 1) / seg : 1;
-    const bool piped = !AG && !B.prof && (n_seg >= 2 || (seg > 0 && getenv("SH_BK_SEG")));
+    const int n_seg = B.n_seg;
     if (piped && !h->bk_side) {
         if (hipStreamCreateWithFlags(&h->bk_side, hipStreamNonBlocking) != hipSuccess) {
             h->bk_side = nullptr;
@@ -1094,11 +1105,10 @@
             return fail(h, SH_E_HIP, what);
         };
         for (int k = 0; k < n_seg; k++) {
-            const int c0 = k * seg, c1 = std::min(c0 + seg, B.n_chunks);
-            B.c0 = c0;
-            B.et0 = c0 * B.ct;
-            B.et1 = std::min(c1 * B.ct, B.nt);
-            if (hipModuleLaunchKernel((hipFunction_t)h->bk.match, (unsigned)(SHB_NB * (c1 - c0)), 1, 1, 512, 1, 1, 0, st,
+            B.c0 = k * B.seg_slots;
+            B.et0 = k * B.seg_tiles;
+            B.et1 = std::min(B.et0 + B.seg_tiles, B.nt);
+            if (hipModuleLaunchKernel((hipFunction_t)h->bk.match, (unsigned)(SHB_NB * bk_seg_slots(B, B.et1 - B.et0)), 1, 1, 512, 1, 1, 0, st,
                                       args, nullptr) != hipSuccess)
                 return quit("shb_match launch failed");
             if (hipEventRecord(h->bk_ev[k], st) != hipSuccess || hipStreamWaitEvent(sd, h->bk_ev[k], 0) != hipSuccess)
@@ -1112,7 +1122,10 @@
             hipStreamWaitEvent(st, h->bk_ev[sh_handle::SH_BK_SEGS], 0) != hipSuccess)
             return quit("bucket join event");
     } else {
-        if (hipModuleLaunchKernel((hipFunction_t)h->bk.match, (unsigned)(SHB_NB * B.n_chunks), 1, 1, 512, 1, 1, 0, st,
+        B.c0 = 0;
+        B.et0 = 0;
+        B.et1 = B.nt;
+        if (hipModuleLaunchKernel((hipFunction_t)h->bk.match, (unsigned)(SHB_NB * bk_seg_slots(B, B.nt)), 1, 1, 512, 1, 1, 0, st,
                                   args, nullptr) != hipSuccess)
             return fail(h, SH_E_HIP, "shb_match launch failed");
         if (AG && shb_agg_carry(&B, AG, st)) return fail(h, SH_E_HIP, "aggregate carry launch failed");
@@ -1161,9 +1174,30 @@
     AG.parallel = mode == BK_AGG_PAR ? 1 : 0;
     if (P.agg_post && !carry && h->out_mode != SHB_OUT_RAW && !h->cols_rows) return 1;
     if (const int wrc = bk_workspace(h, run, kb, true, "bucket workspace", &B)) return wrc;
-    static const int ct_env = getenv("SH_BK_CT") ? atoi(getenv("SH_BK_CT")) : 0;
+    const int ct_env = getenv("SH_BK_CT") ? atoi(getenv("SH_BK_CT")) : 0;
     B.ct = ct_env > 0 ? std::min(ct_env, SHB_CT_MAX) : std::min(shj_bucket_chunk() * 15 / 512, SHB_CT_MAX);
-    B.n_chunks = (B.nt + B.ct - 1) / B.ct;
+    const bool piped = bk_segments(B, carry);
+    shi_pred drop;
+    shi_derive(P, &drop);
+    for (int q = 0; drop.on && q < drop.n_open + drop.n_take; q++) {
+        shi_term& T = q < drop.n_open ? drop.open[q] : drop.take[q - drop.n_open];
+        int k = 0;
+        while (k < h->bk.n_staged && h->bk.staged_attr[k] != T.col) k++;
+        if (k == h->bk.n_staged || B.st_width[k] != T.width) drop.on = 0;
+        T.col = k;
+    }
+    if (const char* e = getenv("SH_BK_DROP"))
+        if (atoi(e) == 0) drop.on = 0;
+    if (carry || B.seg_tiles > 8192) drop.on = 0;
+    const bool drop_refused = drop.on && h->drop_refused;
+    if (drop_refused) drop.on = 0;
+    h->drop_last = 0;
+    B.cut = drop.on;
+    B.span_lim = shj_bucket_chunk();
+    B.seg_slots = bk_seg_slots(B, B.seg_tiles);
+    B.n_chunks = B.n_seg * B.seg_slots;
+    if (h->bk_ctab.ensure_fresh((int64_t)B.n_chunks * 8)) return fail(h, SH_E_OOM, "bucket workspace");
+    B.ctab = h->bk_ctab.as<int32_t>();
     B.within = std::max<int64_t>(0, P.within_ms);
     for (int k = 0; k < B.n_staged; k++) {
         if (h->bk_st[k].ensure_fresh((int64_t)B.nt * SHB_TILE * B.st_width[k])) return fail(h, SH_E_OOM, "bucket workspace");
@@ -1198,8 +1232,8 @@
     hipMemcpyAsync(h->bk_rd.p, run->d_ts, 8, hipMemcpyDeviceToHost, st);
     if (hipStreamSynchronize(st) != hipSuccess) return fail(h, SH_E_HIP, "bucket: timestamp read");
     B.tbase = *h->bk_rd.as<int64_t>() - ((int64_t)1 << (31 - kb));
-    if (const int brc = bk_begin(h, run, nkeys, &B, "bucket partition launch failed")) return brc;
-    if (const int lrc = bucket_launch(h, run, B, O, OC, carry ? &AG : nullptr)) return lrc;
+    if (const int brc = bk_begin(h, run, nkeys, &B, &drop, "bucket partition launch failed")) return brc;
+    if (const int lrc = bucket_launch(h, run, B, O, OC, carry ? &AG : nullptr, piped)) return lrc;
     int32_t flag = 0;
     int64_t total = 0;
     if (const int erc = bk_end(h, &B, "device error in bucket engine", &flag, &total)) return erc;
@@ -1222,7 +1256,12 @@
         h->aggp_refused = res->refused = true;
         return 1;
     }
+    if (drop.on && flag == SHB_F_ORDER) {
+        h->drop_refused = true;
+        return run_bucket(h, run, nkeys, mode, res);
+    }
     const int rc = bk_close(h, run, flag, total, &h->bk_last, "bucket engine");
+    if (h->bk_last) h->drop_last = drop.on ? 1 : (drop_refused ? -1 : 0);
     if (h->bk_last && carry) {
         res->carried = mode;
         h->agg_last = AG.parallel ? 5 : 4;
@@ -1291,7 +1330,7 @@
     for (int o = 0; o < O.n_out; o++) wd[o] = 4;
     direct_layout(h, run, wd, O.n_out, &OC);
     hipStream_t st = h->stream;
-    if (const int brc = bk_begin(h, run, nkeys, &B, "sequence partition failed")) return brc;
+    if (const int brc = bk_begin(h, run, nkeys, &B, nullptr, "sequence partition failed")) return brc;
     if (shb_s3_carry(&B, &S, st)) return fail(h, SH_E_HIP, "sequence carry launch failed");
     if (shb_finish(&B, h->w_scan.as<uint32_t>(), st)) return fail(h, SH_E_HIP, "sequence scan failed");
     hipEventRecord(h->ev[2], st);
diff --git a/siddhi_amd/csrc/sh_host_int.h b/siddhi_amd/csrc/sh_host_int.h
--- a/siddhi_amd/csrc/sh_host_int.h
+++ b/siddhi_amd/csrc/sh_host_int.h
@@ -19,6 +19,7 @@
 #include "../../include/siddhi_hip.h"
 #include "sh_agg.h"
 #include "sh_agg_seq.h"
+#include "sh_bucket_drop.h"
 #include "sh_bucket_plan.h"
 #include "sh_device.h"
 #include "sh_having.h"
@@ -346,6 +347,9 @@
     std::string bk_emit_err;
     int bk_emit_last = 0;
     bool aggp_refused = false;
+    DevBuf bk_ctab;
+    bool drop_refused = false;
+    int drop_last = 0;
     DevBuf w_colrows;
     bool cols_rows = false;
     int out_mode = SHB_OUT_RAW;
@@ -470,6 +474,7 @@
 int shx_jit_status(sh_handle* h);
 int shx_jit_compile(sh_handle* h);
 int shx_bucket_status(sh_handle* h);
+int shx_bucket_drop_status(sh_handle* h);
 int shx_seq3_status(sh_handle* h);
 int shx_agg_status(sh_handle* h);
 int shx_having_status(sh_handle* h);
diff --git a/siddhi_amd/csrc/sh_jit.cpp b/siddhi_amd/csrc/sh_jit.cpp
--- a/siddhi_amd/csrc/sh_jit.cpp
+++ b/siddhi_amd/csrc/sh_jit.cpp
@@ -981,11 +981,14 @@
 // neighbouring segments of a tile share cache lines
 // (the launch holds the chunks from P.c0 on: every global quantity goes by the chunk's
 // index in the step, none by the grid; SHB_NB is a multiple of 8, so the XCD of a
-// block is that of its position in the launch)
+// block is that of its position in the launch). The chunk's tiles [A, E) come from
+// the chunk table (k_bk_prep_b); a launch holds every slot of its segment, and the
+// workgroups of a slot without a chunk return at once
 const uint32_t gbid = (uint32_t)P.c0 * SHB_NB + blockIdx.x;
 const int b = (int)((gbid & 7u) * (SHB_NB / 8) + ((gbid >> 3) & (SHB_NB / 8 - 1)));
-const int A = (int)(gbid / SHB_NB) * P.ct;
-const int E = A + P.ct < P.nt ? A + P.ct : P.nt;
+const int A = P.ctab[2 * (gbid / SHB_NB)];
+const int E = P.ctab[2 * (gbid / SHB_NB) + 1];
+if (A >= E) return;  // (uniform)
 const int kb = P.kb;
 const uint32_t kmask = (1u << kb) - 1u;
 const int lane = (int)(threadIdx.x & 63u), wv = (int)(threadIdx.x >> 6);
@@ -1015,7 +1018,8 @@
     src += R"(// the pass's segments, one per tile from the first halo tile h0: seg_p[t] the
 // events of the bucket before segment t (only differences are used), seg_g[t] the
 // global index of its first event
-const int h0 = tb_h[a - A];
+// (a chunk cut by valid events: the halo bound may reach past the table's first tile)
+const int h0 = tb_h[a - A] > T0 ? tb_h[a - A] : T0;
 const int nseg = E - h0;
 const uint32_t* const seg_p = tb_p + (h0 - T0);
 const uint32_t* const seg_g = tb_g + (h0 - T0);
diff --git a/siddhi_amd/csrc/sh_vm.h b/siddhi_amd/csrc/sh_vm.h
--- a/siddhi_amd/csrc/sh_vm.h
+++ b/siddhi_amd/csrc/sh_vm.h
@@ -2,62 +2,9 @@
 #include <hip/hip_runtime.h>
 
 #include "../../include/sh_query.h"
+#include "sh_cmp.h"
 #include "sh_device.h"
 
-struct VmVal {
-    int64_t b;
-    uint8_t t;
-    uint8_t null;
-};
-
-__device__ __forceinline__ float bits_f32(int64_t b) { return __int_as_float((int32_t)(uint32_t)b); }
-__device__ __forceinline__ double bits_f64(int64_t b) { return __longlong_as_double(b); }
-__device__ __forceinline__ int64_t f32_bits(float f) { return (int64_t)(uint32_t)__float_as_int(f); }
-__device__ __forceinline__ int64_t f64_bits(double d) { return __double_as_longlong(d); }
-
-__device__ __forceinline__ int64_t to_i64(const VmVal& v) {
-    return v.t == SH_T_LONG ? v.b : (int64_t)(int32_t)v.b;
-}
-__device__ __forceinline__ float to_f32(const VmVal& v) {
-    switch (v.t) {
-        case SH_T_INT: return (float)(int32_t)v.b;
-        case SH_T_LONG: return (float)v.b;
-        case SH_T_FLOAT: return bits_f32(v.b);
-        default: return (float)bits_f64(v.b);
-    }
-}
-__device__ __forceinline__ double to_f64(const VmVal& v) {
-    switch (v.t) {
-        case SH_T_INT: return (double)(int32_t)v.b;
-        case SH_T_LONG: return (double)v.b;
-        case SH_T_FLOAT: return (double)bits_f32(v.b);
-        default: return bits_f64(v.b);
-    }
-}
-
-template <typename T>
-__device__ __forceinline__ bool cmp_op(int op, T a, T b) {
-    switch (op) {
-        case SH_OP_EQ: return a == b;
-        case SH_OP_NE: return a != b;
-        case SH_OP_GT: return a > b;
-        case SH_OP_GE: return a >= b;
-        case SH_OP_LT: return a < b;
-        default: return a <= b;
-    }
-}
-
-
-__device__ __forceinline__ bool vm_cmp(int op, int dom, const VmVal& l, const VmVal& r) {
-    switch (dom) {
-        case DOM_I32: return cmp_op<int32_t>(op, (int32_t)l.b, (int32_t)r.b);
-        case DOM_I64: return cmp_op<int64_t>(op, to_i64(l), to_i64(r));
-        case DOM_F32: return cmp_op<float>(op, to_f32(l), to_f32(r));
-        case DOM_F64: return cmp_op<double>(op, to_f64(l), to_f64(r));
-        case DOM_BOOL: return cmp_op<int>(op, l.b != 0, r.b != 0);
-        default: return cmp_op<int32_t>(op, (int32_t)l.b, (int32_t)r.b);
-    }
-}
 
 __device__ __forceinline__ VmVal vm_arith(int aop, int rt, const VmVal& l, const VmVal& r) {
     VmVal o;
diff --git a/siddhi_amd/device_run.py b/siddhi_amd/device_run.py
--- a/siddhi_amd/device_run.py
+++ b/siddhi_amd/device_run.py
@@ -152,6 +152,9 @@
     def bucket_status(self):
         return lib().shx_bucket_status(self.handle.h)
 
+    def bucket_drop_status(self):
+        return lib().shx_bucket_drop_status(self.handle.h)
+
     def bucket_emit_status(self):
         return lib().shx_bucket_emit_status(self.handle.h)
 
```

Measured after the change: 29.32 billion, median of 3. No clear change (+0.2%).
